# Hansard-T/FHE-Linformer

Measured on AMD Instinct MI355X. Metric: encrypted Linformer-d128 forward ms/sample, lower is better.
Workload: dtype u64

## Files before the change

### fhe-linformer_amd/csrc/context.cpp

```cpp
#include "context.h"
#include <hip/hip_runtime.h>
#include <algorithm>
#include <cstdio>
#include <cstdlib>
#include <cstring>
#include <sys/random.h>
#include <time.h>
#include <cxxabi.h>
#include <dlfcn.h>
#include <execinfo.h>

namespace fhelin {

void hip_check(hipError_t e, const char* what) {
    if (e != hipSuccess) throw Error(FHELIN_ERR_HIP, std::string(what) + ": " + hipGetErrorString(e));
}

void* DevicePool::raw_malloc(size_t bytes) {
    if (backend_.malloc_fn) return backend_.malloc_fn(bytes);
    void* p = nullptr;
    if (hipMalloc(&p, bytes) != hipSuccess) {
        (void)hipGetLastError();
        return nullptr;
    }
// ... 115 lines not shown
    sl.free_at.erase(off);
    if (len > bytes) {
        sl.free_at[off + bytes] = len - bytes;
        ln.by_size.emplace(len - bytes, std::make_pair(slab, off + bytes));
    }
    sl.used += bytes;
    void* p = sl.base + off;
    live_[p] = Live{bytes, cur_lane, slab, off};
    live_bytes_ += bytes;
    if (live_bytes_ > live_peak) live_peak = live_bytes_;
    return p;
}
void DevicePool::free(void* p, unsigned used_by_lanes) {
    if (!p) return;
    auto it = live_.find(p);
    if (it == live_.end()) throw Error(FHELIN_ERR_STATE, "DevicePool::free of unknown pointer");
    const Live lv = it->second;
    live_.erase(it);
    live_bytes_ -= lv.bytes;
    Lane& ln = lane_[lv.lane];
    ln.slabs[lv.slab].used -= lv.bytes;
    unsigned wait = used_by_lanes;
    if (have_streams && lv.lane != cur_lane) {
        wait |= 1u << cur_lane;
        if (conservative_foreign_free)
            for (int k = 0; k <= n_user_lanes; ++k) wait |= 1u << k;
    }
    wait &= ~(1u << lv.lane);
    if (!have_streams || !wait) {
        insert_free(ln, lv.slab, lv.off, lv.bytes);
        return;
    }
    Parked pk{lv.slab, lv.off, lv.bytes, {}, 0};
    for (int k = 0; k < MAX_LANES; ++k) {
        if (!(wait & (1u << k)) || !lane_stream[k]) continue;
        hipEvent_t ev = nullptr;
        if (!spare_events_.empty()) {
            ev = spare_events_.back();
            spare_events_.pop_back();
        } else {
            hip_check(hipEventCreateWithFlags(&ev, hipEventDisableTiming), "hipEventCreate(pool)");
        }
        hip_check(hipEventRecord(ev, lane_stream[k]), "hipEventRecord(pool free)");
        pk.ev[pk.n_ev++] = ev;
    }
    foreign_frees += 1;
    ln.parked.push_back(pk);
}
void DevicePool::trim() {
    trims += 1;
    if (!backend_.malloc_fn) (void)hipDeviceSynchronize();
    for (auto& ln : lane_) {
        for (auto& pk : ln.parked) {
            for (int k = 0; k < pk.n_ev; ++k) spare_events_.push_back(pk.ev[k]);
            insert_free(ln, pk.slab, pk.off, pk.len);
        }
        ln.parked.clear();
        for (size_t i = 0; i < ln.slabs.size(); ++i) {
            Slab& sl = ln.slabs[i];
            if (!sl.base || sl.used != 0) continue;
            erase_size_entry(ln, (int)i, 0, sl.size);
            raw_free(sl.base);
            reserved_ -= sl.size;
            sl = Slab();
        }
    }
}

template <class T>
const T* Context::upload_table(const std::vector<T>& v) {
    void* p = nullptr;
    size_t bytes = std::max<size_t>(v.size() * sizeof(T), 16);
    hip_check(hipMalloc(&p, bytes), "hipMalloc(table)");
    if (!v.empty()) hip_check(hipMemcpy(p, v.data(), v.size() * sizeof(T), hipMemcpyHostToDevice), "hipMemcpy(table)");
    table_allocs.push_back(p);
    return static_cast<const T*>(p);
}
template const u64* Context::upload_table<u64>(const std::vector<u64>&);
template const int* Context::upload_table<int>(const std::vector<int>&);
template const u32* Context::upload_table<u32>(const std::vector<u32>&);
template const double* Context::upload_table<double>(const std::vector<double>&);

static u64 mont_r(u64 m) { return (u64)((((u128)1) << 64) % m); }

static u64 prod_mod(const std::vector<u64>& ms, int skip, u64 t) {
    u64 r = 1 % t;
    for (int i = 0; i < (int)ms.size(); ++i)
        if (i != skip) r = h_mulmod(r, ms[i] % t, t);
    return r;
}

static void resolve_seed(Params& p) {
    if (p.have_seed_bytes) return;
    if (p.seed != 0) {
        std::memset(p.seed_bytes, 0, sizeof p.seed_bytes);
        for (int i = 0; i < 8; ++i) p.seed_bytes[i] = (uint8_t)(p.seed >> (8 * i));
    } else {
        size_t got = 0;
        while (got < sizeof p.seed_bytes) {
            const ssize_t n = getrandom(p.seed_bytes + got, sizeof p.seed_bytes - got, 0);
            if (n <= 0) throw Error(FHELIN_ERR_INTERNAL, "getrandom failed: no entropy for key generation");
            got += (size_t)n;
        }
    }
    p.have_seed_bytes = true;
}

static Params resolve_params(Params p) {
    resolve_seed(p);
    if (p.n_p < 0 && p.n_q >= 1 && p.dnum >= 1 && p.special_bits >= 1) {
        const int a = (p.n_q + p.dnum - 1) / p.dnum;
        const int first = p.first_bits + (std::min(a, p.n_q) - 1) * p.scale_bits;
        const int other = p.n_q > a ? std::min(a, p.n_q - a) * p.scale_bits : 0;
        p.n_p = (std::max(first, other) + p.special_bits - 1) / p.special_bits;
    }
    return p;
}

Context::Context(const Params& p_in) : prm(resolve_params(p_in)) {
    const Params& p = prm;
    if (p.log_n < 12 || p.log_n > 17) throw Error(FHELIN_ERR_ARG, "log_n must be in [12,17]");
    if (p.n_q < 1 || p.n_q > 64 || p.n_p < 0 || p.n_p > 16) throw Error(FHELIN_ERR_ARG, "bad limb counts");
    if (p.dnum < 1) throw Error(FHELIN_ERR_ARG, "dnum must be >= 1");
    if (p.first_bits > 60 || p.scale_bits > 60 || p.special_bits > 60) throw Error(FHELIN_ERR_ARG, "primes must be <= 60 bits");
    if (p.first_bits < 20 || p.scale_bits < 20 || (p.n_p > 0 && p.special_bits < 20)) throw Error(FHELIN_ERR_ARG, "primes must be >= 20 bits");
    if (p.log_slots < 1 || p.log_slots > p.log_n - 1) throw Error(FHELIN_ERR_ARG, "log_slots out of range");
    N = 1 << p.log_n;
    L = p.n_q - 1;
    K = p.n_p;
    alpha = (p.n_q + p.dnum - 1) / p.dnum;
    if (alpha > 16) throw Error(FHELIN_ERR_ARG, "digit size > 16 limbs not supported");
    if ((p.n_q + alpha - 1) / alpha > 16) throw Error(FHELIN_ERR_ARG, "more than 16 key-switching digits not supported");
    try {
        chain = make_prime_chain(p.log_n, p.n_q, p.first_bits, p.scale_bits, p.n_p, p.special_bits);
    } catch (const std::exception& e) {
        throw Error(FHELIN_ERR_ARG, std::string("prime chain: ") + e.what());
    }
    moduli = chain.q;
    moduli.insert(moduli.end(), chain.p.begin(), chain.p.end());
    for (u64 q : moduli)
        if (q >> 60) throw Error(FHELIN_ERR_ARG, "prime chain: a modulus is >= 2^60 (lower scale_bits or first_bits)");
    for (u64 q : moduli) {
        barrett.push_back(h_barrett(q));
        tw.push_back(make_twiddles(q, p.log_n));
    }
    sf_real.assign(p.n_q + 1, 0.0L);
    sf_real[0] = (long double)chain.q[L];
    for (int k = 0; k < L; ++k) sf_real[k + 1] = sf_real[k] * sf_real[k] / (long double)chain.q[L - k];

    if (p.device < 0) return;

    int ndev = 0;
    if (hipGetDeviceCount(&ndev) != hipSuccess || ndev <= 0)
        throw Error(FHELIN_ERR_NO_DEVICE, "no HIP device visible: the fhe-linformer_amd engine has no CPU fallback");
    if (p.device >= ndev) throw Error(FHELIN_ERR_ARG, "device index out of range");
    hip_check(hipSetDevice(p.device), "hipSetDevice");
    hip_check(hipStreamCreateWithFlags(&stream, hipStreamNonBlocking), "hipStreamCreate");
    main_stream = stream;
    own_stream = true;
    {
        int want = 2;
        if (const char* e = std::getenv("FHELIN_LANES")) want = std::atoi(e);
        n_lanes = std::max(0, std::min(want, DevicePool::MAX_LANES - 1));
        for (int k = 1; k <= n_lanes; ++k) {
            hip_check(hipStreamCreateWithFlags(&lane_stream[k], hipStreamNonBlocking), "hipStreamCreate(lane)");
            hip_check(hipEventCreateWithFlags(&lane_event[k], hipEventDisableTiming), "hipEventCreate(lane)");
        }
        hip_check(hipEventCreateWithFlags(&fork_event, hipEventDisableTiming), "hipEventCreate(fork)");
        pool.lane_stream[0] = main_stream;
        for (int k = 1; k <= n_lanes; ++k) pool.lane_stream[k] = lane_stream[k];
        pool.have_streams = true;
        if (const char* e = std::getenv("FHELIN_ASYNC")) async_lanes = std::atoi(e) != 0;
        if (const char* e = std::getenv("FHELIN_FUSE_MODDOWN")) fuse_moddown = std::atoi(e) != 0;
        if (const char* e = std::getenv("FHELIN_FUSE_FINISH")) fuse_finish = std::atoi(e) != 0;
        if (const char* e = std::getenv("FHELIN_HOST_ENCODE")) host_encode = std::atoi(e) != 0;
        if (const char* e = std::getenv("FHELIN_FUSE_GATHER")) fuse_gather = std::atoi(e) != 0;
        if (const char* e = std::getenv("FHELIN_FUSE_LIFT")) fuse_lift = std::atoi(e) != 0;
        if (const char* e = std::getenv("FHELIN_LDS_DIGITS")) lds_digits = std::atoi(e) != 0;
        if (const char* e = std::getenv("FHELIN_NTT_TRACE")) trace_small_ntt = std::atoi(e);
        if (const char* e = std::getenv("FHELIN_HOST_WAITS")) trace_waits = std::atoi(e) != 0;
    }
    hip_check(hipEventCreate(&ev_start), "hipEventCreate");
    stage_words = (size_t)2 << p.log_n;
    for (int i = 0; i < STAGE_SLOTS; ++i) {
        hip_check(hipHostMalloc(reinterpret_cast<void**>(&stage_buf[i]), stage_words * sizeof(u64), hipHostMallocDefault), "hipHostMalloc(stage)");
        hip_check(hipEventCreateWithFlags(&stage_ev[i], hipEventDisableTiming), "hipEventCreate(stage)");
    }
    hip_check(hipHostMalloc(reinterpret_cast<void**>(&small_buf), (size_t)SMALL_SLOTS * SMALL_WORDS * sizeof(u64), hipHostMallocDefault), "hipHostMalloc(stage, small)");
    for (int i = 0; i < SMALL_SLOTS; ++i) hip_check(hipEventCreateWithFlags(&small_ev[i], hipEventDisableTiming), "hipEventCreate(stage, small)");
    hip_check(hipEventCreate(&ev_stop), "hipEventCreate");
    has_device = true;

    const int nl = (int)moduli.size();
    {
        std::vector<u64> bar(2 * nl), ninv(8 * nl, 0);
        for (int i = 0; i < nl; ++i) {
            bar[2 * i] = barrett[i].r0;
            bar[2 * i + 1] = barrett[i].r1;
            ninv[8 * i] = tw[i].n_inv;
            ninv[8 * i + 1] = tw[i].n_inv_s;
            ninv[8 * i + 2] = tw[i].w1_n_inv;
            ninv[8 * i + 3] = tw[i].w1_n_inv_s;
            int bits = 0;
            while (bits < 64 && (moduli[i] >> bits)) ++bits;
            if (bits >= 12 && bits <= 60) {
                ninv[8 * i + 4] = (u64)(bits - 10);
                ninv[8 * i + 5] = (u64)((((u128)1) << (bits + 22)) / moduli[i]);
            }
        }
        dt.log_n = p.log_n;
        dt.n_limbs = nl;
        dt.moduli = upload_table(moduli);
        dt.barrett = upload_table(bar);
        {
            std::vector<u64> qi(nl);
            for (int i = 0; i < nl; ++i) {
                u64 x = moduli[i];
                for (int it = 0; it < 6; ++it) x *= 2 - moduli[i] * x;
                qi[i] = x;
            }
            dt.qinv = upload_table(qi);
            std::vector<u64> mr(2 * (size_t)nl);
            for (int i = 0; i < nl; ++i) {
                mr[2 * i] = mont_r(moduli[i]);
                mr[2 * i + 1] = h_shoup(mr[2 * i], moduli[i]);
            }
            dt.mont = upload_table(mr);
        }
        dt.ninv = upload_table(ninv);
        std::vector<u64> f((size_t)nl * 2 * N), g((size_t)nl * 2 * N);
        for (int i = 0; i < nl; ++i) {
            std::memcpy(&f[(size_t)i * 2 * N], tw[i].fwd.data(), sizeof(u64) * 2 * N);
            std::memcpy(&g[(size_t)i * 2 * N], tw[i].inv.data(), sizeof(u64) * 2 * N);
        }
        dt.tw_fwd = upload_table(f);
        dt.tw_inv = upload_table(g);
        const size_t tiles = N >> 12;
        const size_t per_limb = tiles * 15 * 256 * 2;
        for (int dir = 0; dir < 2; ++dir) {
            const std::vector<u64>& src = dir ? g : f;
            std::vector<u64> r((size_t)nl * per_limb);
            for (int i = 0; i < nl; ++i)
                for (size_t T = 0; T < tiles; ++T)
                    for (int kb = 0; kb < 4; ++kb)
                        for (int j = 0; j < (8 >> kb); ++j)
                            for (size_t tau = 0; tau < 256; ++tau) {
                                const size_t idx = (N >> (kb + 1)) + ((((T << 8) | tau)) << (3 - kb)) + j;
                                const size_t s_ = (size_t)(8 >> kb) - 1 + j;
                                const size_t o = (size_t)i * per_limb + ((T * 15 + s_) * 256 + tau) * 2;
                                r[o] = src[(size_t)i * 2 * N + 2 * idx];
                                r[o + 1] = src[(size_t)i * 2 * N + 2 * idx + 1];
                            }
            (dir ? dt.tw_rows_inv : dt.tw_rows_fwd) = upload_table(r);
        }
    }
    {
        std::vector<u64> phatinv(2 * std::max(K, 1)), phatmod((size_t)std::max(K, 1) * (L + 1)), pinv(2 * (L + 1));
        for (int j = 0; j < K; ++j) {
            u64 pj = chain.p[j];
            u64 hat = prod_mod(chain.p, j, pj);
            u64 inv = h_invmod(hat, pj);
            phatinv[2 * j] = inv;
            phatinv[2 * j + 1] = h_shoup(inv, pj);
            for (int t = 0; t <= L; ++t) phatmod[(size_t)j * (L + 1) + t] = pack30(h_mulmod(prod_mod(chain.p, j, chain.q[t]), mont_r(chain.q[t]), chain.q[t]));
        }
        for (int t = 0; t <= L; ++t) {
            u64 qt = chain.q[t];
            u64 pm = prod_mod(chain.p, -1, qt);
            u64 inv = K > 0 ? h_invmod(pm, qt) : 1;
            pinv[2 * t] = inv;
            pinv[2 * t + 1] = h_shoup(inv, qt);
        }
        d_phatinv = upload_table(phatinv);
        d_phatmod = upload_table(phatmod);
        d_pinv = upload_table(pinv);
        std::vector<u64> pmod(2 * (L + 1));
        for (int t = 0; t <= L; ++t) {
            pmod[2 * t] = prod_mod(chain.p, -1, chain.q[t]);
            pmod[2 * t + 1] = h_shoup(pmod[2 * t], chain.q[t]);
        }
        d_pmod = upload_table(pmod);
        std::vector<u64> qlinv((size_t)(L + 1) * (L + 1) * 2, 0), qlmod((size_t)(L + 1) * (L + 1), 0);
        for (int l = 0; l <= L; ++l)
            for (int t = 0; t < l; ++t) {
                u64 qt = chain.q[t];
                u64 r = chain.q[l] % qt;
                u64 inv = h_invmod(r, qt);
                qlmod[(size_t)l * (L + 1) + t] = r;
                qlinv[((size_t)l * (L + 1) + t) * 2] = inv;
                qlinv[((size_t)l * (L + 1) + t) * 2 + 1] = h_shoup(inv, qt);
            }
        d_qlinv = upload_table(qlinv);
        d_qlmod = upload_table(qlmod);
    }
    lvl.resize(L + 2);
    for (int ell = 1; ell <= L + 1; ++ell) {
        LevelTables& lt = lvl[ell];
        lt.ell = ell;
        lt.beta = digits_at(ell);
        const int nt = ell + K;
        std::vector<u64> hatinv(2 * ell), hatmod((size_t)ell * nt, 0), hatmod2((size_t)ell * nt, 0);
        std::vector<int> tab((size_t)lt.beta * nt, -1);
        for (int j = 0; j < lt.beta; ++j) {
            const int lo = j * alpha, hi = std::min((j + 1) * alpha, ell);
            std::vector<u64> dig(chain.q.begin() + lo, chain.q.begin() + hi);
            for (int i = lo; i < hi; ++i) {
                u64 qi = chain.q[i];
                u64 inv = h_invmod(prod_mod(dig, i - lo, qi), qi);
                hatinv[2 * i] = inv;
                hatinv[2 * i + 1] = h_shoup(inv, qi);
                for (int t = 0; t < nt; ++t) {
                    u64 mt = t < ell ? chain.q[t] : chain.p[t - ell];
                    const u64 hr = h_mulmod(prod_mod(dig, i - lo, mt), mont_r(mt), mt);
                    hatmod[(size_t)i * nt + t] = pack30(hr);
                    hatmod2[(size_t)i * nt + t] = pack30(h_mulmod(hr, mont_r(mt), mt));
                }
            }
            for (int t = 0; t < nt; ++t) {
                bool own = t >= lo && t < hi;
                tab[(size_t)j * nt + t] = own ? -1 : (t < ell ? limb_id_q(t) : limb_id_p(t - ell));
            }
        }
        lt.up_hatinv = upload_table(hatinv);
        lt.up_hatmod = upload_table(hatmod);
        lt.up_hatmod_r2 = upload_table(hatmod2);
        lt.ext_limb_tab = upload_table(tab);
        if (ell >= 2 && K >= 1) {
            const u64 ql = chain.q[ell - 1];
            const int e1 = ell - 1;
            std::vector<u64> mhi(2 * (K + 1)), mhm((size_t)(K + 1) * e1), minv(2 * e1), mmod(e1);
            for (int j = 0; j <= K; ++j) {
                const u64 b = j < K ? chain.p[j] : ql;
                const u64 hat_b = j < K ? h_mulmod(prod_mod(chain.p, j, b), ql % b, b) : prod_mod(chain.p, -1, b);
                const u64 inv = h_invmod(hat_b, b);
                mhi[2 * j] = inv;
                mhi[2 * j + 1] = h_shoup(inv, b);
                for (int t = 0; t < e1; ++t) {
                    const u64 qt = chain.q[t];
                    mhm[(size_t)j * e1 + t] = pack30(j < K ? h_mulmod(prod_mod(chain.p, j, qt), ql % qt, qt) : prod_mod(chain.p, -1, qt));
                }
            }
            for (int t = 0; t < e1; ++t) {
                const u64 qt = chain.q[t];
                mmod[t] = h_mulmod(prod_mod(chain.p, -1, qt), ql % qt, qt);
                const u64 inv = h_invmod(mmod[t], qt);
                minv[2 * t] = inv;
                minv[2 * t + 1] = h_shoup(inv, qt);
            }
            lt.md_hatinv = upload_table(mhi);
            lt.md_hatmod = upload_table(mhm);
            lt.md_minv = upload_table(minv);
            lt.md_mmod = upload_table(mmod);
        }
    }
}

void Context::upload_async(u64* dst, const u64* src, size_t words) {
    if (words <= SMALL_WORDS && small_buf) {
        const int i = small_next;
        small_next = (small_next + 1) % SMALL_SLOTS;
        if (small_used[i]) {
            timespec a, b;
            if (trace_waits) clock_gettime(CLOCK_MONOTONIC, &a);
            hip_check(hipEventSynchronize(small_ev[i]), "hipEventSynchronize(stage, small)");
            if (trace_waits) {
                clock_gettime(CLOCK_MONOTONIC, &b);
                note_wait("upload ring (small)", (u64)((b.tv_sec - a.tv_sec) * 1000000000ll + (b.tv_nsec - a.tv_nsec)));
            }
        }
        u64* slot = small_buf + (size_t)i * SMALL_WORDS;
        std::memcpy(slot, src, words * sizeof(u64));
        hip_check(hipMemcpyAsync(dst, slot, words * sizeof(u64), hipMemcpyHostToDevice, stream), "hipMemcpyAsync(stage, small)");
        hip_check(hipEventRecord(small_ev[i], stream), "hipEventRecord(stage, small)");
        small_used[i] = true;
        return;
    }
    if (words > stage_words) throw Error(FHELIN_ERR_INTERNAL, "upload_async: block larger than a staging slot");
    const int i = stage_next;
    stage_next = (stage_next + 1) % STAGE_SLOTS;
    if (stage_used[i]) {
        timespec a, b;
        if (trace_waits) clock_gettime(CLOCK_MONOTONIC, &a);
        hip_check(hipEventSynchronize(stage_ev[i]), "hipEventSynchronize(stage)");
        if (trace_waits) {
            clock_gettime(CLOCK_MONOTONIC, &b);
            note_wait("upload ring (large)", (u64)((b.tv_sec - a.tv_sec) * 1000000000ll + (b.tv_nsec - a.tv_nsec)));
        }
    }
    std::memcpy(stage_buf[i], src, words * sizeof(u64));
    hip_check(hipMemcpyAsync(dst, stage_buf[i], words * sizeof(u64), hipMemcpyHostToDevice, stream), "hipMemcpyAsync(stage)");
    hip_check(hipEventRecord(stage_ev[i], stream), "hipEventRecord(stage)");
    stage_used[i] = true;
}

Context::~Context() {
    if (trace_waits) {
        fprintf(stderr, "[fhelin] host time blocked inside the library, by site (waits, ms):\n");
        for (const auto& e : wait_sites) fprintf(stderr, "  %8llu %10.1f  %s\n", (unsigned long long)e.second.first, e.second.second / 1e6, e.first.c_str());
    }
    if (trace_small_ntt && !small_ntt_sites.empty()) {
        std::vector<std::pair<std::string, std::pair<u64, u64>>> v(small_ntt_sites.begin(), small_ntt_sites.end());
        std::sort(v.begin(), v.end(), [](const auto& a, const auto& b) { return a.second.first > b.second.first; });
        fprintf(stderr, "[fhelin] transforms of <= %d limb vectors by call stack (launch pairs, limb vectors):\n", trace_small_ntt);
        for (size_t i = 0; i < v.size() && i < 40; ++i)
            fprintf(stderr, "  %8llu %9llu  %s\n", (unsigned long long)v[i].second.first, (unsigned long long)v[i].second.second, v[i].first.c_str());
    }
    if (has_device) {
        (void)hipSetDevice(prm.device);
        (void)hipDeviceSynchronize();
        for (void* p : table_allocs) (void)hipFree(p);
        for (int k = 1; k <= n_lanes; ++k) {
            if (lane_event[k]) (void)hipEventDestroy(lane_event[k]);
            if (lane_stream[k]) (void)hipStreamDestroy(lane_stream[k]);
        }
        if (fork_event) (void)hipEventDestroy(fork_event);
        for (int i = 0; i < STAGE_SLOTS; ++i) {
            if (stage_ev[i]) (void)hipEventDestroy(stage_ev[i]);
            if (stage_buf[i]) (void)hipHostFree(stage_buf[i]);
        }
        for (int i = 0; i < SMALL_SLOTS; ++i)
            if (small_ev[i]) (void)hipEventDestroy(small_ev[i]);
        if (small_buf) (void)hipHostFree(small_buf);
        if (ev_start) (void)hipEventDestroy(ev_start);
        if (ev_stop) (void)hipEventDestroy(ev_stop);
        if (own_stream && main_stream) (void)hipStreamDestroy(main_stream);
    }
}

void Context::require_device() const {
    if (!has_device)
        throw Error(FHELIN_ERR_NO_DEVICE, "operation needs the HIP device path (host-only context): no CPU fallback exists");
}
// ... 106 lines not shown
```

### fhe-linformer_amd/csrc/context.h

```cpp
#pragma once
#include <cstdint>
#include <map>
#include <memory>
#include <stdexcept>
#include <string>
#include <unordered_map>
#include <vector>
#include <hip/hip_runtime_api.h>
#include "../../include/fhelin.h"
#include "hostmath.h"
#include "kernels.h"

namespace fhelin {

struct Params {
    int log_n = 16;
    int n_q = 24;
    int first_bits = 55;
    int scale_bits = 52;
    int n_p = 6;
    int special_bits = 60;
    int dnum = 4;
    int log_slots = 14;
    int hamming = 192;
    uint64_t seed = 0;
    uint8_t seed_bytes[32] = {};
    bool have_seed_bytes = false;
    int device = 0;
};

struct Error : std::runtime_error {
    int code;
    Error(int c, const std::string& m) : std::runtime_error(m), code(c) {}
};

void hip_check(hipError_t e, const char* what);

class DevicePool {
public:
    static constexpr int MAX_LANES = 5;
    static constexpr size_t SLAB_MAX = size_t(8) << 30, SLAB_MIN = size_t(32) << 20;
    struct Backend {
        void* (*malloc_fn)(size_t) = nullptr;
        void (*free_fn)(void*) = nullptr;
    };
    DevicePool() = default;
    explicit DevicePool(const Backend& b) : backend_(b) {}
    ~DevicePool();
    void* alloc(size_t bytes);
    void free(void* p, unsigned used_by_lanes = 0);
    bool conservative_foreign_free = false;
    int n_user_lanes = 0;
    void trim();
    size_t bytes_reserved() const { return reserved_; }
    size_t bytes_live() const { return live_bytes_; }
    size_t slabs() const;
    size_t free_ranges() const;
    int cur_lane = 0;
    hipStream_t lane_stream[MAX_LANES] = {};
    bool have_streams = false;
    u64 malloc_calls = 0, malloc_bytes = 0, malloc_ns = 0;
    u64 foreign_frees = 0;
    u64 trims = 0;
    size_t live_peak = 0, reserved_peak = 0;
private:
    struct Slab {
        char* base = nullptr;
        size_t size = 0, used = 0;
        std::map<size_t, size_t> free_at;
    };
    struct Live { size_t bytes; int lane; int slab; size_t off; };
    struct Parked { int slab; size_t off, len; hipEvent_t ev[MAX_LANES]; int n_ev; };
    struct Lane {
        std::vector<Slab> slabs;
        std::multimap<size_t, std::pair<int, size_t>> by_size;
        std::vector<Parked> parked;
    };
    Backend backend_;
    Lane lane_[MAX_LANES];
    std::unordered_map<void*, Live> live_;
    std::vector<hipEvent_t> spare_events_;
    size_t reserved_ = 0, live_bytes_ = 0;
    void insert_free(Lane& ln, int slab, size_t off, size_t len);
    void erase_size_entry(Lane& ln, int slab, size_t off, size_t len);
    bool grow(Lane& ln, size_t bytes);
    void* raw_malloc(size_t bytes);
    void raw_free(void* p);
};

struct LevelTables {
    int ell = 0;
    int beta = 0;
    const u64* up_hatinv = nullptr;
    const u64* up_hatmod = nullptr;
    const u64* up_hatmod_r2 = nullptr;
    const int* ext_limb_tab = nullptr;
    const u64* md_hatinv = nullptr;
    const u64* md_hatmod = nullptr;
    const u64* md_minv = nullptr;
    const u64* md_mmod = nullptr;
};

struct OpStats {
    u64 limb_ntt = 0;
    u64 keyswitch = 0;
    u64 keyswitch_limbs = 0;
    u64 rescale = 0;
    u64 ct_pt_mult = 0;
    u64 bootstrap = 0;
    u64 encode = 0;
    u64 rescale_limbs = 0;
    u64 ct_pt_limbs = 0;
};

struct Context {
    Params prm;
    OpStats stats;
    int N = 0;
    int L = 0;
    int K = 0;
    int alpha = 0;
    PrimeChain chain;
    std::vector<u64> moduli;
    std::vector<Barrett> barrett;
    std::vector<TwiddleTable> tw;
    std::vector<long double> sf_real;

    bool has_device = false;
    hipStream_t stream = nullptr;
    hipStream_t main_stream = nullptr;
    bool own_stream = false;
    int n_lanes = 0;
    hipStream_t lane_stream[DevicePool::MAX_LANES] = {};
    hipEvent_t lane_event[DevicePool::MAX_LANES] = {};
    hipEvent_t fork_event = nullptr;
    bool async_lanes = true;
    int async_rr = 0;
    u64 lane_seq[DevicePool::MAX_LANES] = {};
    std::vector<std::pair<u64, std::shared_ptr<void>>> lane_hold[DevicePool::MAX_LANES];
    void release_holds(int lane, u64 up_to_seq);
    void fork_lanes();
    void join_lanes();
    struct LaneScope {
        Context& c;
        LaneScope(Context& ctx, int k) : c(ctx) {
            c.stream = c.lane_stream[k];
            c.pool.cur_lane = k;
        }
        ~LaneScope() {
            c.stream = c.main_stream;
            c.pool.cur_lane = 0;
        }
    };
    DevicePool pool;
    DeviceTables dt{};
    std::vector<void*> table_allocs;
    hipEvent_t ev_start = nullptr, ev_stop = nullptr;

    static constexpr int STAGE_SLOTS = 64;
    u64* stage_buf[STAGE_SLOTS] = {};
    hipEvent_t stage_ev[STAGE_SLOTS] = {};
    bool stage_used[STAGE_SLOTS] = {};
    int stage_next = 0;
    size_t stage_words = 0;
    static constexpr int SMALL_SLOTS = 256;
    static constexpr size_t SMALL_WORDS = 8192;
    u64* small_buf = nullptr;
    hipEvent_t small_ev[SMALL_SLOTS] = {};
    bool small_used[SMALL_SLOTS] = {};
    int small_next = 0;
    void upload_async(u64* dst, const u64* src, size_t words);

    const u64* d_phatinv = nullptr;
    const u64* d_phatmod = nullptr;
    const u64* d_pinv = nullptr;
    const u64* d_pmod = nullptr;
    const u64* d_qlinv = nullptr;
    const u64* d_qlmod = nullptr;
    std::vector<LevelTables> lvl;
    std::map<u64, const u32*> automorph_maps;

    explicit Context(const Params& p);
    ~Context();
    Context(const Context&) = delete;
    Context& operator=(const Context&) = delete;

    void require_device() const;
    template <class T> T* dalloc(size_t count) { return static_cast<T*>(pool.alloc(count * sizeof(T))); }
    template <class T> const T* upload_table(const std::vector<T>& v);
    int limb_id_q(int i) const { return i; }
    int limb_id_p(int j) const { return L + 1 + j; }
    int digits_at(int ell) const { return (ell + alpha - 1) / alpha; }
    u64 galois_element(int rot_index) const;
    const u32* automorph_map(u64 galois);
    const u32* automorph_inverse_of(const u32* map);
    std::map<const u32*, const u32*> automorph_inverse;
    bool fuse_finish = true;
    bool fuse_moddown = false;
    bool host_encode = false;
    bool fuse_gather = true;
    bool fuse_lift = true;
    bool lds_digits = true;
    struct FftDev {
        const u32* rot = nullptr;
        const double* ksi = nullptr;
    };
    std::map<int, FftDev> fft_dev;
    void sync();
    void ntt(const LimbBatch& b, bool inverse, int active = -1) {
        stats.limb_ntt += (u64)(active >= 0 ? active : b.nvec);
        if (trace_small_ntt && b.nvec <= trace_small_ntt) note_small_ntt(b.nvec);
        launch_ntt(dt, b, inverse, stream);
    }
    bool trace_waits = false;
    std::map<std::string, std::pair<u64, u64>> wait_sites;
    void note_wait(const char* site, u64 ns) {
        auto& e = wait_sites[site];
        e.first += 1;
        e.second += ns;
    }
    int trace_small_ntt = 0;
    std::map<std::string, std::pair<u64, u64>> small_ntt_sites;
    void note_small_ntt(int nvec);
    void ntt_epilogue(const LimbBatch& b, const NttEpilogue& ep) {
        stats.limb_ntt += (u64)b.nvec;
        if (trace_small_ntt && b.nvec <= trace_small_ntt) note_small_ntt(b.nvec);
        launch_ntt_epilogue(dt, b, ep, stream);
    }
};

}
```

### fhe-linformer_amd/csrc/evaluator.cpp

```cpp
#include "evaluator.h"
#include <map>
#include <hip/hip_runtime.h>
#include <cmath>
#include <cstring>

namespace fhelin {

DevBlock::~DevBlock() {
    if (d && ctx) {
        try { ctx->pool.free(d); } catch (...) {}
    }
}
Ciphertext::~Ciphertext() {
    if (async_ev) (void)hipEventDestroy(async_ev);
    if (d && ctx && !block) {
        try { ctx->pool.free(d); } catch (...) {}
    }
}
Encoding::~Encoding() {
    if (ready) (void)hipEventDestroy(ready);
    if (d && ctx) {
        try { ctx->pool.free(d, lanes_ordered); } catch (...) {}
    }
}
// ... 61 lines not shown

std::vector<CtPtr> Evaluator::make_contiguous(const std::vector<CtPtr>& v, int site) {
    if (v.size() <= 1 || contiguous_base(v)) return v;
    if (site >= 0 && site < 8) gather_copies[site] += v.size();
    std::vector<CtPtr> o = new_ct_batch((int)v.size(), v[0]->npoly, v[0]->ell, v[0]->deg, v[0]->scale, v[0]->slots);
    for (size_t lo = 0; lo < v.size(); lo += EwItems::MAX_ITEMS) {
        EwItems it;
        it.n = (int)std::min<size_t>(EwItems::MAX_ITEMS, v.size() - lo);
        it.vecs = v[0]->npoly * v[0]->ell;
        it.b_vecs = 0;
        for (int i = 0; i < it.n; ++i) {
            if (v[lo + i]->words() != v[0]->words()) throw Error(FHELIN_ERR_INTERNAL, "make_contiguous: operands of different shapes");
            it.out[i] = o[lo + i]->d;
            it.a[i] = v[lo + i]->d;
            it.b[i] = nullptr;
        }
        launch_ew_items(c_.dt, it, 4, v[0]->ell, c_.stream);
    }
    hip_check(hipGetLastError(), "batch gather");
    return o;
}

KeyPtr Evaluator::new_key() {
    c_.require_device();
    auto k = std::make_shared<EvalKey>();
    k->ctx = &c_;
    k->digits = c_.digits_at(c_.L + 1);
    k->d = c_.dalloc<u64>(k->words());
    return k;
}

void Evaluator::keyswitch(const u64* c_ntt, int ell, const EvalKey& key, u64* out, const u64* add0, const u64* add1,
                          const u32* map, const u64* post) {
    keyswitch_batch(1, c_ntt, 0, ell, key, out, 0, add0, add1, 0, map, post, 0);
}

void Evaluator::keyswitch_batch(int B, const u64* c_ntt, size_t c_stride, int ell, const EvalKey& key, u64* out, size_t out_stride,
                                const u64* add0, const u64* add1, size_t add_stride, const u32* map, const u64* post,
                                size_t post_stride) {
    keyswitch_impl(B, nullptr, c_ntt, c_stride, ell, &key, out, out_stride, add0, add1, add_stride, map, post, post_stride);
}

void Evaluator::keyswitch_rows(const KsRows& rows, const u64* c_ntt, size_t c_stride, int ell, u64* out, size_t out_stride,
                               const u64* add0, size_t add_stride) {
    const int B = (int)rows.keys.size();
    if (B < 1) return;
    if (B > KsShape::MAX_ROWS || rows.maps.size() != rows.keys.size()) throw Error(FHELIN_ERR_ARG, "keyswitch_rows: bad row count");
    keyswitch_impl(B, &rows, c_ntt, c_stride, ell, nullptr, out, out_stride, add0, nullptr, add_stride, nullptr, nullptr, 0);
}

void Evaluator::keyswitch_impl(int B, const KsRows* rows, const u64* c_ntt, size_t c_stride, int ell, const EvalKey* key, u64* out,
                               size_t out_stride, const u64* add0, const u64* add1, size_t add_stride, const u32* map, const u64* post,
                               size_t post_stride) {
    c_.require_device();
    if (c_.K < 1) throw Error(FHELIN_ERR_STATE, "hybrid key switching needs at least one special prime");
    if (B < 1) return;
    const size_t N = c_.N;
    const int K = c_.K, L1 = c_.L + 1;
    const LevelTables& lt = c_.lvl[ell];
    const int nt = ell + K;
    KsShape sh{ell, K, c_.alpha, lt.beta, L1, B, c_stride, out_stride, add_stride, post_stride};
    const bool shared = rows && rows->shared_input;
    if (rows) {
        sh.per_row = 1;
        sh.shared_input = shared ? 1 : 0;
        for (int b = 0; b < B; ++b) {
            sh.evk_row[b] = rows->keys[b]->d;
            sh.map_row[b] = rows->maps[b];
        }
    }
    const int Bu = shared ? 1 : B;
    KsShape shu = sh;
    shu.batch = Bu;
    hipStream_t s = c_.stream;
    u64* cc = c_.dalloc<u64>((size_t)Bu * ell * N);
    c_.stats.keyswitch += (u64)B;
    c_.stats.keyswitch_limbs += (u64)B * ell;
    {
        LimbBatch ib{cc, Bu * ell, nullptr, 0, ell, c_ntt};
        if (Bu > 1 && c_stride != (size_t)ell * N) {
            ib.src_group = ell;
            ib.src_group_stride = c_stride;
        }
        c_.ntt(ib, true);
    }
    u64* ext = c_.dalloc<u64>((size_t)Bu * lt.beta * nt * N);
    launch_modup_conv(c_.dt, shu, ext, cc, c_ntt, lt.up_hatinv, lt.up_hatmod_r2, s);
    LimbBatch eb{ext, Bu * lt.beta * nt, lt.ext_limb_tab, 0, 1};
    eb.tab_len = lt.beta * nt;
    eb.lazy_out = true;
    c_.ntt(eb, false, Bu * (lt.beta * nt - ell));
    u64* accQ = c_.dalloc<u64>((size_t)B * 2 * ell * N);
    u64* accP = c_.dalloc<u64>((size_t)B * 2 * K * N);
    launch_ks_inner(c_.dt, sh, accQ, accP, ext, key ? key->d : nullptr, c_ntt, s);
    c_.ntt(LimbBatch{accP, B * 2 * K, nullptr, L1, K}, true);
    u64* conv = c_.dalloc<u64>((size_t)B * 2 * ell * N);
    launch_moddown_conv(c_.dt, sh, conv, accP, c_.d_phatinv, c_.d_phatmod, s);
    const bool identity = !map && !rows;
    if (c_.fuse_moddown || (c_.fuse_finish && identity)) {
        NttEpilogue ep;
        ep.acc = accQ;
        ep.acc_poly_stride = (size_t)ell * N;
        ep.out = out;
        ep.out_stride = out_stride;
        ep.w = c_.d_pinv;
        ep.ell = ell;
        ep.add0 = add0;
        ep.add1 = add1;
        ep.add_stride = add_stride;
        ep.post = post;
        ep.post_stride = post_stride;
        if (rows) {
            ep.per_row = 1;
            for (int b = 0; b < B; ++b) ep.invmap_row[b] = c_.automorph_inverse_of(rows->maps[b]);
        } else if (map) {
            ep.invmap = c_.automorph_inverse_of(map);
        }
        c_.ntt_epilogue(LimbBatch{conv, B * 2 * ell, nullptr, 0, ell}, ep);
    } else {
        c_.ntt(LimbBatch{conv, B * 2 * ell, nullptr, 0, ell}, false);
        launch_moddown_finish(c_.dt, sh, out, accQ, conv, c_.d_pinv, add0, add1, map, post, s);
    }
    launch_ok("keyswitch");
    c_.pool.free(cc);
    c_.pool.free(ext);
    c_.pool.free(accQ);
    c_.pool.free(accP);
    c_.pool.free(conv);
}

void Evaluator::moddown_rescale_finish(const KsShape& sh, u64* out, const u64* accQ, u64* conv, const u64* minv) {
    const int e1 = sh.ell - 1;
    const LimbBatch cb{conv, sh.batch * 2 * e1, nullptr, 0, e1};
    if (c_.fuse_finish) {
        NttEpilogue ep;
        ep.acc = accQ;
        ep.acc_poly_stride = (size_t)sh.ell * c_.N;
        ep.out = out;
        ep.out_stride = sh.out_stride;
        ep.w = minv;
        ep.ell = e1;
        c_.ntt_epilogue(cb, ep);
        return;
    }
    c_.ntt(cb, false);
    launch_moddown_rescale_finish(c_.dt, sh, out, accQ, conv, minv, c_.stream);
}

bool Evaluator::have_rotation_keys(const std::vector<int>& indices, int slots) const {
    const int ns = slots > 0 ? slots : (1 << c_.prm.log_slots);
    for (int r : indices) {
        if (r % ns == 0) return false;
        if (!rot_keys.count(c_.galois_element(r))) return false;
    }
    return !indices.empty();
}

const u64* Evaluator::permuted(const EvalKey& key, const u32* map) {
    if (key.d_perm) return key.d_perm;
    const int nvec = key.digits * 2 * (c_.L + 1 + c_.K);
    key.d_perm = c_.dalloc<u64>(key.words());
    launch_automorph_pack30(c_.dt, key.d_perm, key.d, map, nvec, c_.stream);
    launch_ok("key permutation");
    hip_check(hipStreamSynchronize(c_.stream), "key permutation sync");
    return key.d_perm;
}

std::vector<CtPtr> Evaluator::rotate_sum_batch(const std::vector<CtPtr>& vin, const std::vector<int>& indices) {
    if (vin.empty()) return {};
    const int R = (int)indices.size();
    if (R < 1 || R > KsShape::MAX_ROT) throw Error(FHELIN_ERR_ARG, "rotate_sum_batch: 1..7 rotations");
    if (!have_rotation_keys(indices, vin[0]->slots)) throw Error(FHELIN_ERR_KEY, "rotate_sum_batch: missing rotation key");
    if (c_.K < 1) throw Error(FHELIN_ERR_STATE, "hybrid key switching needs at least one special prime");
    std::vector<const EvalKey*> keys;
    std::vector<const u32*> maps;
    for (int r : indices) {
        const u64 g = c_.galois_element(r);
        keys.push_back(rot_keys.at(g).get());
        maps.push_back(c_.automorph_map(g));
    }
    const size_t N = c_.N;
    const int K = c_.K, L1 = c_.L + 1;
    hipStream_t s = c_.stream;
    std::vector<CtPtr> out(vin.size());
    std::vector<char> done(vin.size(), 0);
    for (size_t first = 0; first < vin.size(); ++first) {
        if (done[first]) continue;
        if (vin[first]->npoly != 2) throw Error(FHELIN_ERR_STATE, "rotate: ciphertext must have 2 components");
        std::vector<size_t> idx;
        for (size_t i = first; i < vin.size() && (int)idx.size() < batch_limit; ++i) {
            const CtPtr &a = vin[first], &b = vin[i];
            if (!done[i] && b->npoly == 2 && b->ell == a->ell && b->deg == a->deg && fabsl(b->scale / a->scale - 1.0L) < 1e-9L)
                idx.push_back(i);
        }
        std::vector<CtPtr> chunk;
        for (size_t i : idx) chunk.push_back(vin[i]);
        chunk = make_contiguous(chunk, 0);
        const int B = (int)chunk.size(), ell = chunk[0]->ell;
        const size_t pn = (size_t)ell * N, ctw = 2 * pn;
        const LevelTables& lt = c_.lvl[ell];
        const int nt = ell + K;
        std::vector<CtPtr> o = new_ct_batch(B, 2, ell, chunk[0]->deg, chunk[0]->scale, chunk[0]->slots);
        const u64* base = chunk[0]->d;
        KsShape sh{ell, K, c_.alpha, lt.beta, L1, B, ctw, ctw, pn, ctw};
        sh.n_rot = R;
        sh.lds_digits = c_.lds_digits ? 1 : 0;
        for (int r = 0; r < R; ++r) {
            sh.evk_rot[r] = permuted(*keys[r], maps[r]);
            sh.map_rot[r] = maps[r];
            if (c_.galois_element(indices[r]) % (u64)(c_.N / 256) != 1) sh.lds_digits = 0;
        }
        int steps = 0;
        while ((1 << steps) < R + 1) ++steps;
        c_.stats.keyswitch += (u64)B * steps;
        c_.stats.keyswitch_limbs += (u64)B * steps * ell;
        u64* cc = c_.dalloc<u64>((size_t)B * ell * N);
        {
            LimbBatch ib{cc, B * ell, nullptr, 0, ell, base + pn};
            if (B > 1) {
                ib.src_group = ell;
                ib.src_group_stride = ctw;
            }
            c_.ntt(ib, true);
        }
        u64* ext = c_.dalloc<u64>((size_t)B * lt.beta * nt * N);
        launch_modup_conv(c_.dt, sh, ext, cc, base + pn, lt.up_hatinv, lt.up_hatmod, s);
        LimbBatch eb{ext, B * lt.beta * nt, lt.ext_limb_tab, 0, 1};
        eb.tab_len = lt.beta * nt;
        eb.lazy_out = true;
        c_.ntt(eb, false, B * (lt.beta * nt - ell));
        u64* accQ = c_.dalloc<u64>((size_t)B * 2 * ell * N);
        u64* accP = c_.dalloc<u64>((size_t)B * 2 * K * N);
        launch_ks_inner_multi(c_.dt, sh, accQ, accP, ext, base + pn, s);
        u64* c0sum = nullptr;
        if (c_.fuse_gather) {
            sh.gsrc = base;
            sh.gsrc_stride = ctw;
        } else {
            c0sum = c_.dalloc<u64>((size_t)B * ell * N);
            launch_gather_sum(c_.dt, sh, c0sum, base, ctw, s);
        }
        c_.ntt(LimbBatch{accP, B * 2 * K, nullptr, L1, K}, true);
        u64* conv = c_.dalloc<u64>((size_t)B * 2 * ell * N);
        launch_moddown_conv(c_.dt, sh, conv, accP, c_.d_phatinv, c_.d_phatmod, s);
        c_.ntt(LimbBatch{conv, B * 2 * ell, nullptr, 0, ell}, false);
        launch_moddown_finish(c_.dt, sh, o[0]->d, accQ, conv, c_.d_pinv, c0sum, nullptr, nullptr, base, s);
        launch_ok("rotate_sum_batch");
        c_.pool.free(cc);
        c_.pool.free(ext);
        c_.pool.free(accQ);
        c_.pool.free(accP);
        if (c0sum) c_.pool.free(c0sum);
        c_.pool.free(conv);
        for (int b = 0; b < B; ++b) {
            o[b]->scale = vin[idx[b]]->scale;
            out[idx[b]] = o[b];
            done[idx[b]] = 1;
        }
    }
    return out;
}

Evaluator::FoldedKey Evaluator::folded_key(const PtPtr& p, int index, long double scale) {
    const u64 g = c_.galois_element(index);
    auto kit = rot_keys.find(g);
    if (kit == rot_keys.end()) throw Error(FHELIN_ERR_KEY, "no rotation key for index " + std::to_string(index) + " (EvalRotateKeyGen list)");
    for (size_t i = 0; i < folded_keys.size(); ++i) {
        const FoldedKey& f = folded_keys[i];
        if (f.pt.get() == p.get() && f.key.get() == kit->second.get() && f.index == index && f.scale == scale) {
            FoldedKey hit = f;
            if (i + 1 != folded_keys.size()) {
                folded_keys.erase(folded_keys.begin() + i);
                folded_keys.push_back(hit);
            }
            return hit;
        }
    }
    FoldedKey f;
    f.pt = p;
    f.key = kit->second;
    f.index = index;
    f.scale = scale;
    const int nl = c_.L + 1 + c_.K;
    f.enc = p->at(nl, scale);
    f.d = std::make_shared<DevBlock>();
    f.d->ctx = &c_;
    f.d->d = c_.dalloc<u64>(f.key->words());
    launch_fold_key(c_.dt, f.d->d, f.key->d, c_.automorph_map(g), f.enc->d, f.key->digits * 2 * nl, c_.stream);
    launch_ok("fold_key");
    hip_check(hipStreamSynchronize(c_.stream), "fold_key sync");
    if (folded_keys.size() >= MAX_FOLDED) {
        hip_check(hipStreamSynchronize(c_.main_stream), "folded key eviction sync");
        for (int k = 1; k <= c_.n_lanes; ++k) hip_check(hipStreamSynchronize(c_.lane_stream[k]), "folded key eviction sync (lane)");
        folded_keys.erase(folded_keys.begin());
    }
    folded_keys.push_back(f);
    return f;
}

std::vector<CtPtr> Evaluator::hoisted_dot_rows(const std::vector<CtPtr>& xin, const std::vector<PtPtr>& pts, const std::vector<int>& indices,
                                              bool rescale_out) {
    if (xin.empty()) return {};
    const int R = (int)indices.size();
    if (R < 1 || R > KsShape::MAX_ROT || (int)pts.size() != R + 1)
        throw Error(FHELIN_ERR_ARG, "hoisted_dot_rows: 1..7 rotations, one plaintext per rotation + the unrotated term's");
    if (!have_rotation_keys(indices, xin[0]->slots)) throw Error(FHELIN_ERR_KEY, "hoisted_dot_rows: missing rotation key");
    if (c_.K < 1) throw Error(FHELIN_ERR_STATE, "hybrid key switching needs at least one special prime");
    const int ns = xin[0]->slots > 0 ? xin[0]->slots : (1 << c_.prm.log_slots);
    for (int r : indices)
        if (r % ns == 0) throw Error(FHELIN_ERR_ARG, "hoisted_dot_rows: a rotation by 0 is the unrotated term (pts[0])");
    if (rescale_out && c_.K + 1 > 16)
        return rescale_batch(hoisted_dot_rows(xin, pts, indices, false));
    std::vector<CtPtr> x = xin;
    {
        std::vector<CtPtr> need;
        std::vector<size_t> pos;
        for (size_t i = 0; i < x.size(); ++i)
            if (x[i]->deg >= 2) {
                need.push_back(x[i]);
                pos.push_back(i);
            }
        if (!need.empty()) {
            std::vector<CtPtr> r = rescale_batch(need);
            for (size_t k = 0; k < pos.size(); ++k) x[pos[k]] = r[k];
        }
    }
    std::vector<const u32*> maps;
    for (int r : indices) maps.push_back(c_.automorph_map(c_.galois_element(r)));
    const size_t N = c_.N;
    const int K = c_.K, L1 = c_.L + 1;
    hipStream_t s = c_.stream;
    std::vector<CtPtr> out(x.size());
    std::vector<char> done(x.size(), 0);
    for (size_t first = 0; first < x.size(); ++first) {
        if (done[first]) continue;
        if (x[first]->npoly != 2) throw Error(FHELIN_ERR_STATE, "hoisted_dot_rows: ciphertext must have 2 components");
        std::vector<size_t> idx;
        for (size_t i = first; i < x.size() && (int)idx.size() < batch_limit; ++i) {
            const CtPtr &a = x[first], &b = x[i];
            if (!done[i] && b->npoly == 2 && b->ell == a->ell && b->deg == a->deg && fabsl(b->scale / a->scale - 1.0L) < 1e-9L) idx.push_back(i);
        }
        std::vector<CtPtr> chunk;
        for (size_t i : idx) chunk.push_back(x[i]);
        chunk = make_contiguous(chunk, 0);
        const int B = (int)chunk.size(), ell = chunk[0]->ell;
        const size_t pn = (size_t)ell * N, ctw = 2 * pn;
        const LevelTables& lt = c_.lvl[ell];
        const int nt = ell + K;
        const long double sf = c_.sf_real[chunk[0]->level()];
        const bool merged = rescale_out && ell >= 2 && K + 1 <= 16;
        if (rescale_out && !merged) throw Error(FHELIN_ERR_STATE, "hoisted_dot_rows: no limb left to drop");
        const int oell = merged ? ell - 1 : ell;
        std::vector<CtPtr> o = new_ct_batch(B, 2, oell, merged ? chunk[0]->deg : chunk[0]->deg + 1, chunk[0]->scale * sf, chunk[0]->slots);
        const u64* base = chunk[0]->d;
        KsShape sh{ell, K, c_.alpha, lt.beta, L1, B, ctw, (size_t)2 * oell * N, pn, ctw};
        sh.n_rot = R;
        sh.lds_digits = c_.lds_digits ? 1 : 0;
        HoistAdd h;
        h.n_rot = R;
        std::vector<FoldedKey> hold;
        const std::shared_ptr<Encoding> e0 = pts[0]->at(ell, sf);
        h.v[0] = e0->d;
        for (int r = 0; r < R; ++r) {
            hold.push_back(folded_key(pts[r + 1], indices[r], sf));
            sh.evk_rot[r] = hold.back().d->d;
            sh.map_rot[r] = maps[r];
            h.v[r + 1] = hold.back().enc->d;
            h.map[r] = maps[r];
            if (c_.galois_element(indices[r]) % (u64)(c_.N / 256) != 1) sh.lds_digits = 0;
        }
        c_.stats.keyswitch += (u64)B * R;
        c_.stats.keyswitch_limbs += (u64)B * R * ell;
        c_.stats.ct_pt_mult += (u64)B * (R + 1);
        c_.stats.ct_pt_limbs += (u64)B * (R + 1) * ell;
        if (merged) {
            c_.stats.rescale += (u64)B;
            c_.stats.rescale_limbs += (u64)B * ell;
        }
        u64* cc = c_.dalloc<u64>((size_t)B * ell * N);
        {
            LimbBatch ib{cc, B * ell, nullptr, 0, ell, base + pn};
            if (B > 1) {
                ib.src_group = ell;
                ib.src_group_stride = ctw;
            }
            c_.ntt(ib, true);
        }
        u64* ext = c_.dalloc<u64>((size_t)B * lt.beta * nt * N);
        launch_modup_conv(c_.dt, sh, ext, cc, base + pn, lt.up_hatinv, lt.up_hatmod, s);
        LimbBatch eb{ext, B * lt.beta * nt, lt.ext_limb_tab, 0, 1};
        eb.tab_len = lt.beta * nt;
        eb.lazy_out = true;
        c_.ntt(eb, false, B * (lt.beta * nt - ell));
        u64* accQ = c_.dalloc<u64>((size_t)B * 2 * ell * N);
        u64* accP = c_.dalloc<u64>((size_t)B * 2 * K * N);
        launch_ks_inner_multi(c_.dt, sh, accQ, accP, ext, base + pn, s);
        u64* pre = nullptr;
        u64* conv = nullptr;
        u64* top = nullptr;
        if (!merged) {
            pre = c_.dalloc<u64>((size_t)B * ctw);
            launch_hoist_addends(c_.dt, sh, h, pre, base, s);
            c_.ntt(LimbBatch{accP, B * 2 * K, nullptr, L1, K}, true);
            conv = c_.dalloc<u64>((size_t)B * 2 * ell * N);
            launch_moddown_conv(c_.dt, sh, conv, accP, c_.d_phatinv, c_.d_phatmod, s);
            c_.ntt(LimbBatch{conv, B * 2 * ell, nullptr, 0, ell}, false);
            launch_moddown_finish(c_.dt, sh, o[0]->d, accQ, conv, c_.d_pinv, nullptr, nullptr, nullptr, pre, s);
        } else {
            h.acc = accQ;
            h.pmod = c_.d_pmod;
            launch_hoist_addends(c_.dt, sh, h, nullptr, base, s);
            c_.ntt(LimbBatch{accP, B * 2 * K, nullptr, L1, K}, true);
            top = c_.dalloc<u64>((size_t)B * 2 * N);
            {
                LimbBatch tb{top, B * 2, nullptr, ell - 1, 1, accQ + (size_t)(ell - 1) * N};
                tb.src_group = 1;
                tb.src_group_stride = pn;
                c_.ntt(tb, true);
            }
            conv = c_.dalloc<u64>((size_t)B * 2 * (ell - 1) * N);
            launch_moddown_rescale_conv(c_.dt, sh, conv, accP, top, lt.md_hatinv, lt.md_hatmod, lt.md_mmod, s);
            moddown_rescale_finish(sh, o[0]->d, accQ, conv, lt.md_minv);
        }
        launch_ok("hoisted_dot_rows");
        c_.pool.free(cc);
        c_.pool.free(ext);
        c_.pool.free(accQ);
        c_.pool.free(accP);
        if (pre) c_.pool.free(pre);
        if (top) c_.pool.free(top);
        c_.pool.free(conv);
        for (int b = 0; b < B; ++b) {
            o[b]->scale = x[idx[b]]->scale * sf;
            if (merged) o[b]->scale = o[b]->scale / (long double)c_.chain.q[ell - 1];
            out[idx[b]] = o[b];
            done[idx[b]] = 1;
        }
    }
    return out;
}

CtPtr Evaluator::rotate_each_sum(const std::vector<CtPtr>& vin, const std::vector<int>& indices) {
    if (vin.empty() || vin.size() != indices.size()) throw Error(FHELIN_ERR_ARG, "rotate_each_sum: one index per ciphertext");
    const int ns = vin[0]->slots > 0 ? vin[0]->slots : (1 << c_.prm.log_slots);
    std::vector<CtPtr> rot;
    std::vector<int> ridx;
    CtPtr acc;
    for (size_t i = 0; i < vin.size(); ++i) {
        if (indices[i] % ns == 0) acc = acc ? add(acc, vin[i]) : vin[i];
        else {
            rot.push_back(vin[i]);
            ridx.push_back(indices[i]);
        }
    }
    for (size_t first = 0; first < rot.size(); first += KsShape::MAX_ROT) {
        const int R = (int)std::min(rot.size() - first, (size_t)KsShape::MAX_ROT);
        std::vector<CtPtr> chunk(rot.begin() + first, rot.begin() + first + R);
        bool uniform = have_rotation_keys(std::vector<int>(ridx.begin() + first, ridx.begin() + first + R), ns) && c_.K >= 1;
        for (const CtPtr& c : chunk)
            uniform = uniform && c->npoly == 2 && c->ell == chunk[0]->ell && c->deg == chunk[0]->deg &&
                      fabsl(c->scale / chunk[0]->scale - 1.0L) < 1e-9L;
        if (!uniform || R < 2) {
            for (int r = 0; r < R; ++r) {
                CtPtr t = rotate(chunk[r], ridx[first + r]);
                acc = acc ? add(acc, t) : t;
            }
            continue;
        }
        chunk = make_contiguous(chunk, 1);
        const size_t N = c_.N;
        const int K = c_.K, L1 = c_.L + 1, ell = chunk[0]->ell;
        const size_t pn = (size_t)ell * N, ctw = 2 * pn;
        const LevelTables& lt = c_.lvl[ell];
        const int nt = ell + K;
        hipStream_t s = c_.stream;
        const u64* base = chunk[0]->d;
        KsShape up{ell, K, c_.alpha, lt.beta, L1, R, ctw, 0, 0, 0};
        u64* cc = c_.dalloc<u64>((size_t)R * ell * N);
        {
            LimbBatch ib{cc, R * ell, nullptr, 0, ell, base + pn};
            ib.src_group = ell;
            ib.src_group_stride = ctw;
            c_.ntt(ib, true);
        }
        u64* ext = c_.dalloc<u64>((size_t)R * lt.beta * nt * N);
        launch_modup_conv(c_.dt, up, ext, cc, base + pn, lt.up_hatinv, lt.up_hatmod, s);
        LimbBatch eb{ext, R * lt.beta * nt, lt.ext_limb_tab, 0, 1};
        eb.tab_len = lt.beta * nt;
        eb.lazy_out = true;
        c_.ntt(eb, false, R * (lt.beta * nt - ell));
        KsShape sh{ell, K, c_.alpha, lt.beta, L1, 1, 0, ctw, pn, 0};
        sh.n_rot = R;
        sh.rot_ext_stride = (size_t)lt.beta * nt * N;
        sh.rot_input_stride = ctw;
        for (int r = 0; r < R; ++r) {
            const u64 g = c_.galois_element(ridx[first + r]);
            sh.map_rot[r] = c_.automorph_map(g);
            sh.evk_rot[r] = permuted(*rot_keys.at(g), sh.map_rot[r]);
        }
        c_.stats.keyswitch += (u64)R;
        c_.stats.keyswitch_limbs += (u64)R * ell;
        u64* accQ = c_.dalloc<u64>((size_t)2 * ell * N);
        u64* accP = c_.dalloc<u64>((size_t)2 * K * N);
        launch_ks_inner_multi(c_.dt, sh, accQ, accP, ext, base + pn, s);
        u64* c0sum = nullptr;
        if (c_.fuse_gather) {
            sh.gsrc = base;
            sh.gsrc_stride = 0;
        } else {
            c0sum = c_.dalloc<u64>((size_t)ell * N);
            launch_gather_sum(c_.dt, sh, c0sum, base, 0, s);
        }
        c_.ntt(LimbBatch{accP, 2 * K, nullptr, L1, K}, true);
        u64* conv = c_.dalloc<u64>((size_t)2 * ell * N);
        launch_moddown_conv(c_.dt, sh, conv, accP, c_.d_phatinv, c_.d_phatmod, s);
        c_.ntt(LimbBatch{conv, 2 * ell, nullptr, 0, ell}, false);
        CtPtr o = new_ct(2, ell, chunk[0]->deg, chunk[0]->scale, chunk[0]->slots);
        launch_moddown_finish(c_.dt, sh, o->d, accQ, conv, c_.d_pinv, c0sum, nullptr, nullptr, nullptr, s);
        launch_ok("rotate_each_sum");
        c_.pool.free(cc);
        c_.pool.free(ext);
        c_.pool.free(accQ);
        c_.pool.free(accP);
        if (c0sum) c_.pool.free(c0sum);
        c_.pool.free(conv);
        acc = acc ? add(acc, o) : o;
    }
    return acc;
}

std::vector<CtPtr> Evaluator::rotate_each_sum_rows(const std::vector<std::vector<CtPtr>>& rows, const std::vector<int>& indices) {
    if (rows.empty()) return {};
    const int ns = rows[0][0]->slots > 0 ? rows[0][0]->slots : (1 << c_.prm.log_slots);
    std::vector<int> rot_pos, plain_pos, ridx;
    for (size_t r = 0; r < indices.size(); ++r) {
        if (indices[r] % ns == 0) plain_pos.push_back((int)r);
        else {
            rot_pos.push_back((int)r);
            ridx.push_back(indices[r]);
        }
    }
    const int R = (int)rot_pos.size();
    bool uniform = R >= 2 && R <= KsShape::MAX_ROT && have_rotation_keys(ridx, ns) && c_.K >= 1;
    const CtPtr& f = rows[0][0];
    for (const auto& row : rows) {
        uniform = uniform && row.size() == indices.size();
        for (const CtPtr& c : row)
            uniform = uniform && c->npoly == 2 && c->ell == f->ell && c->deg == f->deg && fabsl(c->scale / f->scale - 1.0L) < 1e-9L;
    }
    std::vector<CtPtr> out(rows.size());
    if (!uniform) {
        for (size_t b = 0; b < rows.size(); ++b) out[b] = rotate_each_sum(rows[b], indices);
        return out;
    }
    const size_t N = c_.N;
    const int K = c_.K, L1 = c_.L + 1, ell = f->ell;
    const size_t pn = (size_t)ell * N, ctw = 2 * pn;
    const LevelTables& lt = c_.lvl[ell];
    const int nt = ell + K;
    hipStream_t s = c_.stream;
    const size_t chunk_rows = (size_t)std::max(1, batch_limit / 2);
    for (size_t lo = 0; lo < rows.size(); lo += chunk_rows) {
        const size_t hi = std::min(rows.size(), lo + chunk_rows);
        const int B = (int)(hi - lo);
        std::vector<CtPtr> flat;
        for (size_t b = lo; b < hi; ++b)
            for (int r : rot_pos) flat.push_back(rows[b][r]);
        size_t row_stride = (size_t)R * ctw;
        bool regular = B >= 1 && flat[0]->block != nullptr;
        for (int b = 0; b < B && regular; ++b) {
            for (int r = 0; r < R && regular; ++r) {
                const CtPtr& c = flat[(size_t)b * R + r];
                regular = c->block == flat[0]->block && c->words() == (size_t)ctw &&
                          c->d == flat[(size_t)b * R]->d + (size_t)r * ctw;
            }
            if (regular && b == 1) {
                regular = flat[R]->d > flat[0]->d;
                if (regular) row_stride = (size_t)(flat[R]->d - flat[0]->d);
            }
            if (regular && b >= 1) regular = flat[(size_t)b * R]->d == flat[0]->d + (size_t)b * row_stride;
        }
        if (!regular) {
            flat = make_contiguous(flat, 2);
            row_stride = (size_t)R * ctw;
        }
        const u64* base = flat[0]->d;
        KsShape up{ell, K, c_.alpha, lt.beta, L1, B * R, ctw, 0, 0, 0};
        u64* cc = c_.dalloc<u64>((size_t)B * R * ell * N);
        {
            LimbBatch ib{cc, B * R * ell, nullptr, 0, ell, base + pn};
            ib.src_group = ell;
            ib.src_group_stride = ctw;
            if (row_stride != (size_t)R * ctw) {
                ib.src_group2 = R;
                ib.src_group2_stride = row_stride;
            }
            c_.ntt(ib, true);
        }
        u64* ext = c_.dalloc<u64>((size_t)B * R * lt.beta * nt * N);
        launch_modup_conv(c_.dt, up, ext, cc, base + pn, lt.up_hatinv, lt.up_hatmod, s);
        LimbBatch eb{ext, B * R * lt.beta * nt, lt.ext_limb_tab, 0, 1};
        eb.tab_len = lt.beta * nt;
        eb.lazy_out = true;
        c_.ntt(eb, false, B * R * (lt.beta * nt - ell));
        KsShape sh{ell, K, c_.alpha, lt.beta, L1, B, row_stride, ctw, pn, 0};
        sh.n_rot = R;
        sh.rot_ext_stride = (size_t)lt.beta * nt * N;
        sh.rot_input_stride = ctw;
        sh.ext_batch_stride = (size_t)R * lt.beta * nt * N;
        for (int r = 0; r < R; ++r) {
            const u64 g = c_.galois_element(ridx[r]);
            sh.map_rot[r] = c_.automorph_map(g);
            sh.evk_rot[r] = permuted(*rot_keys.at(g), sh.map_rot[r]);
        }
        sh.gsrc = base;
        sh.gsrc_stride = row_stride;
        c_.stats.keyswitch += (u64)B * R;
        c_.stats.keyswitch_limbs += (u64)B * R * ell;
        u64* accQ = c_.dalloc<u64>((size_t)B * 2 * ell * N);
        u64* accP = c_.dalloc<u64>((size_t)B * 2 * K * N);
        launch_ks_inner_multi(c_.dt, sh, accQ, accP, ext, base + pn, s);
        c_.ntt(LimbBatch{accP, B * 2 * K, nullptr, L1, K}, true);
        u64* conv = c_.dalloc<u64>((size_t)B * 2 * ell * N);
        launch_moddown_conv(c_.dt, sh, conv, accP, c_.d_phatinv, c_.d_phatmod, s);
        c_.ntt(LimbBatch{conv, B * 2 * ell, nullptr, 0, ell}, false);
        std::vector<CtPtr> o = new_ct_batch(B, 2, ell, f->deg, f->scale, f->slots);
        launch_moddown_finish(c_.dt, sh, o[0]->d, accQ, conv, c_.d_pinv, nullptr, nullptr, nullptr, nullptr, s);
        launch_ok("rotate_each_sum_rows");
        c_.pool.free(cc);
        c_.pool.free(ext);
        c_.pool.free(accQ);
        c_.pool.free(accP);
        c_.pool.free(conv);
        for (int b = 0; b < B; ++b) out[lo + b] = o[b];
    }
    if (!plain_pos.empty()) {
        std::vector<CtPtr> acc(rows.size());
        for (size_t b = 0; b < rows.size(); ++b) acc[b] = rows[b][plain_pos[0]];
        for (size_t k = 1; k < plain_pos.size(); ++k) {
            std::vector<CtPtr> t(rows.size());
            for (size_t b = 0; b < rows.size(); ++b) t[b] = rows[b][plain_pos[k]];
            acc = add_batch(acc, t);
        }
        out = add_batch(acc, out);
    }
    return out;
}

std::vector<CtPtr> Evaluator::rotate_many(const CtPtr& a, const std::vector<int>& indices) {
    if (a->npoly != 2) throw Error(FHELIN_ERR_STATE, "rotate: ciphertext must have 2 components");
    const int ns = a->slots > 0 ? a->slots : (1 << c_.prm.log_slots);
    std::vector<CtPtr> out(indices.size());
    std::vector<size_t> todo;
    for (size_t i = 0; i < indices.size(); ++i) {
        if (indices[i] % ns == 0) out[i] = a;
        else todo.push_back(i);
    }
    const size_t pn = (size_t)a->ell * c_.N, ctw = 2 * pn;
    for (size_t first = 0; first < todo.size(); first += KsShape::MAX_ROWS) {
        const int B = (int)std::min(todo.size() - first, (size_t)KsShape::MAX_ROWS);
        if (B == 1) {
            out[todo[first]] = rotate(a, indices[todo[first]]);
            continue;
        }
        KsRows rows;
        rows.shared_input = true;
        for (int b = 0; b < B; ++b) {
            const int index = indices[todo[first + b]];
            const u64 g = c_.galois_element(index);
            auto it = rot_keys.find(g);
            if (it == rot_keys.end())
                throw Error(FHELIN_ERR_KEY, "no rotation key for index " + std::to_string(index) + " (EvalRotateKeyGen list)");
            rows.keys.push_back(it->second.get());
            rows.maps.push_back(c_.automorph_map(g));
        }
        std::vector<CtPtr> o = new_ct_batch(B, 2, a->ell, a->deg, a->scale, a->slots);
        keyswitch_rows(rows, a->d + pn, 0, a->ell, o[0]->d, ctw, a->d, 0);
        for (int b = 0; b < B; ++b) out[todo[first + b]] = o[b];
    }
    return out;
}

std::vector<CtPtr> Evaluator::rotate_each(const std::vector<CtPtr>& vin, const std::vector<int>& indices) {
    if (vin.size() != indices.size()) throw Error(FHELIN_ERR_ARG, "rotate_each: one index per ciphertext");
    std::vector<CtPtr> out(vin.size());
    std::vector<char> done(vin.size(), 0);
    for (size_t first = 0; first < vin.size(); ++first) {
        if (done[first]) continue;
        const CtPtr& a = vin[first];
        if (a->npoly != 2) throw Error(FHELIN_ERR_STATE, "rotate: ciphertext must have 2 components");
        const int ns = a->slots > 0 ? a->slots : (1 << c_.prm.log_slots);
        if (indices[first] % ns == 0) {
            out[first] = clone(a);
            done[first] = 1;
            continue;
        }
        std::vector<size_t> idx;
        for (size_t i = first; i < vin.size() && (int)idx.size() < std::min(batch_limit, (int)KsShape::MAX_ROWS); ++i) {
            const CtPtr& b = vin[i];
            if (!done[i] && indices[i] % ns != 0 && b->npoly == 2 && b->ell == a->ell && b->deg == a->deg &&
                fabsl(b->scale / a->scale - 1.0L) < 1e-9L)
                idx.push_back(i);
        }
        if (idx.size() < 2) {
            out[first] = rotate(a, indices[first]);
            done[first] = 1;
            continue;
// ... 124 lines not shown
    const u32* map = c_.automorph_map(g);
    std::vector<char> done(vin.size(), 0);
    for (size_t first = 0; first < vin.size(); ++first) {
        if (done[first]) continue;
        if (vin[first]->npoly != 2) throw Error(FHELIN_ERR_STATE, "rotate: ciphertext must have 2 components");
        std::vector<size_t> idx;
        for (size_t i = first; i < vin.size() && (int)idx.size() < batch_limit; ++i) {
            const CtPtr &a = vin[first], &b = vin[i];
            if (!done[i] && b->npoly == 2 && b->ell == a->ell && b->deg == a->deg && fabsl(b->scale / a->scale - 1.0L) < 1e-9L)
                idx.push_back(i);
        }
        std::vector<CtPtr> chunk;
        for (size_t i : idx) chunk.push_back(vin[i]);
        chunk = make_contiguous(chunk, 4);
        const int B = (int)chunk.size();
        const int ell = chunk[0]->ell;
        const size_t pn = (size_t)ell * c_.N, ctw = 2 * pn;
        std::vector<CtPtr> o = new_ct_batch(B, 2, ell, chunk[0]->deg, chunk[0]->scale, chunk[0]->slots);
        const u64* base = chunk[0]->d;
        keyswitch_batch(B, base + pn, ctw, ell, key, o[0]->d, ctw, base, nullptr, ctw, map, accumulate ? base : nullptr, ctw);
        for (int b = 0; b < B; ++b) {
            o[b]->scale = vin[idx[b]]->scale;
            out[idx[b]] = o[b];
            done[idx[b]] = 1;
        }
    }
    return out;
}

std::vector<std::vector<CtPtr>> Evaluator::rotate_many_batch(const std::vector<CtPtr>& xs, const std::vector<int>& indices) {
    std::vector<std::vector<CtPtr>> out(xs.size());
    if (xs.empty()) return out;
    bool uniform = xs.size() >= 2 && !c_.fuse_moddown && c_.K >= 1;
    for (const CtPtr& x : xs)
        uniform = uniform && x->npoly == 2 && x->ell == xs[0]->ell && x->deg == xs[0]->deg && x->slots == xs[0]->slots;
    if (!uniform) {
        for (size_t i = 0; i < xs.size(); ++i) out[i] = rotate_many(xs[i], indices);
        return out;
    }
    const int ns = xs[0]->slots > 0 ? xs[0]->slots : (1 << c_.prm.log_slots);
    std::vector<size_t> todo;
    for (size_t i = 0; i < xs.size(); ++i) out[i].resize(indices.size());
    for (size_t k = 0; k < indices.size(); ++k) {
        if (indices[k] % ns == 0)
            for (size_t i = 0; i < xs.size(); ++i) out[i][k] = xs[i];
        else
            todo.push_back(k);
    }
    const int R = (int)todo.size();
    if (R == 0) return out;
    std::vector<const EvalKey*> keys;
    std::vector<const u32*> maps;
    for (size_t k : todo) {
        const u64 g = c_.galois_element(indices[k]);
        auto it = rot_keys.find(g);
        if (it == rot_keys.end())
            throw Error(FHELIN_ERR_KEY, "no rotation key for index " + std::to_string(indices[k]) + " (EvalRotateKeyGen list)");
        keys.push_back(it->second.get());
        maps.push_back(c_.automorph_map(g));
    }
    const size_t N = c_.N;
    const int K = c_.K, L1 = c_.L + 1, ell = xs[0]->ell;
    const size_t pn = (size_t)ell * N, ctw = 2 * pn;
    const LevelTables& lt = c_.lvl[ell];
    const int nt = ell + K;
    hipStream_t s = c_.stream;
    const size_t per_pass = (size_t)std::max(1, 160 / R);
    for (size_t lo = 0; lo < xs.size(); lo += per_pass) {
        const size_t hi = std::min(xs.size(), lo + per_pass);
        const int B = (int)(hi - lo);
        std::vector<CtPtr> in = make_contiguous(std::vector<CtPtr>(xs.begin() + lo, xs.begin() + hi), 6);
        const u64* base = in[0]->d;
        const int rows = B * R;
        c_.stats.keyswitch += (u64)rows;
        c_.stats.keyswitch_limbs += (u64)rows * ell;
        KsShape up{ell, K, c_.alpha, lt.beta, L1, B, ctw, 0, 0, 0};
        u64* cc = c_.dalloc<u64>((size_t)B * ell * N);
        {
            LimbBatch ib{cc, B * ell, nullptr, 0, ell, base + pn};
            if (B > 1) {
                ib.src_group = ell;
                ib.src_group_stride = ctw;
            }
            c_.ntt(ib, true);
        }
        u64* ext = c_.dalloc<u64>((size_t)B * lt.beta * nt * N);
        launch_modup_conv(c_.dt, up, ext, cc, base + pn, lt.up_hatinv, lt.up_hatmod_r2, s);
        LimbBatch eb{ext, B * lt.beta * nt, lt.ext_limb_tab, 0, 1};
        eb.tab_len = lt.beta * nt;
        eb.lazy_out = true;
        c_.ntt(eb, false, B * (lt.beta * nt - ell));
        u64* accQ = c_.dalloc<u64>((size_t)rows * 2 * ell * N);
        u64* accP = c_.dalloc<u64>((size_t)rows * 2 * K * N);
        auto row_shape = [&](int first, int cnt) {
            KsShape sh{ell, K, c_.alpha, lt.beta, L1, B * cnt, ctw, ctw, ctw, 0};
            sh.per_row = 1;
            sh.shared_input = 1;
            sh.row_mod = cnt;
            sh.ext_batch_stride = (size_t)lt.beta * nt * N;
            for (int b = 0; b < cnt; ++b) {
                sh.evk_row[b] = keys[first + b]->d;
                sh.map_row[b] = maps[first + b];
            }
            return sh;
        };
        const bool one_chunk = R <= (int)KsShape::MAX_ROWS;
        if (one_chunk) launch_ks_inner(c_.dt, row_shape(0, R), accQ, accP, ext, nullptr, base + pn, s);
        else
            for (int i = 0; i < B; ++i)
                for (int first = 0; first < R; first += KsShape::MAX_ROWS) {
                    const int cnt = std::min(R - first, (int)KsShape::MAX_ROWS);
                    const size_t row0 = (size_t)i * R + first;
                    KsShape sh1{ell, K, c_.alpha, lt.beta, L1, cnt, 0, ctw, 0, 0};
                    sh1.per_row = 1;
                    sh1.shared_input = 1;
                    for (int b = 0; b < cnt; ++b) {
                        sh1.evk_row[b] = keys[first + b]->d;
                        sh1.map_row[b] = maps[first + b];
                    }
                    launch_ks_inner(c_.dt, sh1, accQ + row0 * 2 * ell * N, accP + row0 * 2 * K * N, ext + (size_t)i * lt.beta * nt * N, nullptr,
                                    base + pn + (size_t)i * ctw, s);
                }
        KsShape dn{ell, K, c_.alpha, lt.beta, L1, rows, 0, ctw, 0, 0};
        c_.ntt(LimbBatch{accP, rows * 2 * K, nullptr, L1, K}, true);
        u64* conv = c_.dalloc<u64>((size_t)rows * 2 * ell * N);
        launch_moddown_conv(c_.dt, dn, conv, accP, c_.d_phatinv, c_.d_phatmod, s);
        c_.ntt(LimbBatch{conv, rows * 2 * ell, nullptr, 0, ell}, false);
        std::vector<CtPtr> o = new_ct_batch(rows, 2, ell, xs[lo]->deg, xs[lo]->scale, xs[lo]->slots);
        if (one_chunk) {
            launch_moddown_finish(c_.dt, row_shape(0, R), o[0]->d, accQ, conv, c_.d_pinv, base, nullptr, nullptr, nullptr, s);
        } else {
            for (int i = 0; i < B; ++i)
                for (int first = 0; first < R; first += KsShape::MAX_ROWS) {
                    const int cnt = std::min(R - first, (int)KsShape::MAX_ROWS);
                    const size_t row0 = (size_t)i * R + first;
                    KsShape sh1{ell, K, c_.alpha, lt.beta, L1, cnt, 0, ctw, 0, 0};
                    sh1.per_row = 1;
                    sh1.shared_input = 1;
                    for (int b = 0; b < cnt; ++b) {
                        sh1.evk_row[b] = keys[first + b]->d;
                        sh1.map_row[b] = maps[first + b];
                    }
                    launch_moddown_finish(c_.dt, sh1, o[row0]->d, accQ + row0 * 2 * ell * N, conv + row0 * 2 * ell * N, c_.d_pinv,
                                          base + (size_t)i * ctw, nullptr, nullptr, nullptr, s);
                }
        }
        launch_ok("rotate_many_batch");
        c_.pool.free(cc);
        c_.pool.free(ext);
        c_.pool.free(accQ);
        c_.pool.free(accP);
        c_.pool.free(conv);
        for (int i = 0; i < B; ++i)
            for (int r = 0; r < R; ++r) {
                o[(size_t)i * R + r]->scale = xs[lo + i]->scale;
                out[lo + i][todo[r]] = o[(size_t)i * R + r];
            }
    }
    return out;
}

std::vector<CtPtr> Evaluator::rescale_batch(const std::vector<CtPtr>& vin) {
    std::vector<CtPtr> out(vin.size());
    std::vector<char> done(vin.size(), 0);
    for (size_t first = 0; first < vin.size(); ++first) {
        if (done[first]) continue;
        std::vector<size_t> idx;
        for (size_t i = first; i < vin.size() && (int)idx.size() < batch_limit; ++i)
            if (!done[i] && vin[i]->npoly == 2 && vin[first]->npoly == 2 && vin[i]->ell == vin[first]->ell) idx.push_back(i);
        if (idx.size() < 2) {
            out[first] = rescale(vin[first]);
            done[first] = 1;
            continue;
        }
        std::vector<CtPtr> chunk;
        for (size_t i : idx) chunk.push_back(vin[i]);
        chunk = make_contiguous(chunk, 5);
        const int B = (int)chunk.size(), ell = chunk[0]->ell, P = 2 * B;
        if (ell < 2) throw Error(FHELIN_ERR_STATE, "rescale: no limb left to drop");
        const size_t N = c_.N;
        const u64* base = chunk[0]->d;
        u64* last = c_.dalloc<u64>((size_t)P * N);
        c_.stats.rescale += (u64)B;
        c_.stats.rescale_limbs += (u64)B * ell;
        LimbBatch lb{last, P, nullptr, ell - 1, 1, base + (size_t)(ell - 1) * N};
        lb.src_group = 1;
        lb.src_group_stride = (size_t)ell * N;
        c_.ntt(lb, true);
        std::vector<CtPtr> o = new_ct_batch(B, 2, ell - 1, 1, 0, chunk[0]->slots);
        rescale_finish(o[0]->d, base, last, P, ell);
        launch_ok("rescale_batch");
        c_.pool.free(last);
        for (int b = 0; b < B; ++b) {
            const CtPtr& a = vin[idx[b]];
            o[b]->scale = a->scale / (long double)c_.chain.q[ell - 1];
            o[b]->deg = a->deg > 1 ? a->deg - 1 : 1;
            out[idx[b]] = o[b];
            done[idx[b]] = 1;
        }
    }
    return out;
}

std::vector<CtPtr> Evaluator::mult_plain_batch(const std::vector<CtPtr>& vin, const PtPtr& p) {
    return mult_plain_each(vin, std::vector<PtPtr>(vin.size(), p));
}

namespace {
template <class SameShape, class Emit>
// ... 60 lines not shown
    if (vin.size() != p.size() || vin.empty()) throw Error(FHELIN_ERR_ARG, "dot_plain: one plaintext per ciphertext, at least one term");
    std::vector<CtPtr> x = vin;
    {
        std::vector<CtPtr> need;
        std::map<const Ciphertext*, size_t> slot;
        for (size_t i = 0; i < vin.size(); ++i)
            if (vin[i]->deg >= 2 && !slot.count(vin[i].get())) {
                slot[vin[i].get()] = need.size();
                need.push_back(vin[i]);
            }
        if (!need.empty()) {
            std::vector<CtPtr> r = rescale_batch(need);
            for (size_t i = 0; i < vin.size(); ++i)
                if (vin[i]->deg >= 2) x[i] = r[slot[vin[i].get()]];
        }
    }
    bool uniform = x.size() >= 2;
    for (const CtPtr& c : x)
        uniform = uniform && c->npoly == x[0]->npoly && c->ell == x[0]->ell && c->deg == x[0]->deg && fabsl(c->scale / x[0]->scale - 1.0L) < 1e-9L;
    if (!uniform) {
        if (pt_scale > 0) throw Error(FHELIN_ERR_ARG, "dot_plain: an explicit plaintext scale needs uniform operands");
        std::vector<CtPtr> prod = mult_plain_each(x, p);
        CtPtr acc = prod[0];
        for (size_t i = 1; i < prod.size(); ++i) acc = add(acc, prod[i]);
        return acc;
    }
    const CtPtr& f = x[0];
    const long double sf = pt_scale > 0 ? pt_scale : c_.sf_real[f->level()];
    CtPtr acc;
    for (size_t lo = 0; lo < x.size(); lo += EwItems::MAX_ITEMS) {
        const size_t hi = std::min(x.size(), lo + (size_t)EwItems::MAX_ITEMS);
        EwItems it;
        it.n = (int)(hi - lo);
        it.vecs = f->npoly * f->ell;
        it.b_vecs = f->ell;
        for (size_t i = lo; i < hi; ++i) {
            it.a[i - lo] = x[i]->d;
            it.b[i - lo] = p[i]->at(f->ell, sf)->d;
        }
        const bool into_dest = dest && x.size() <= (size_t)EwItems::MAX_ITEMS && dest->npoly == f->npoly && dest->ell == f->ell;
        CtPtr o = into_dest ? dest : new_ct(f->npoly, f->ell, f->deg + 1, f->scale * sf, f->slots);
        if (into_dest) {
            o->deg = f->deg + 1;
            o->scale = f->scale * sf;
            o->slots = f->slots;
        }
        launch_ew_dot(c_.dt, o->d, it, f->ell, c_.stream);
        c_.stats.ct_pt_mult += (u64)(hi - lo);
        c_.stats.ct_pt_limbs += (u64)(hi - lo) * f->ell;
        acc = acc ? add(acc, o) : o;
    }
    launch_ok("dot_plain");
    return acc;
}

bool Evaluator::dot_plain_groups(const std::vector<CtPtr>& cts, const std::vector<std::vector<PtPtr>>& pts, long double pt_scale,
                                 const std::vector<CtPtr>& dest) {
    if (!dot_groups || cts.empty() || cts.size() > (size_t)EwDotGroups::MAX_A || pts.empty() || pts.size() > (size_t)EwDotGroups::MAX_G ||
        dest.size() != pts.size())
        return false;
    const CtPtr& f = cts[0];
    for (const CtPtr& c : cts)
        if (c->npoly != 2 || c->deg != 1 || c->ell != f->ell || fabsl(c->scale / f->scale - 1.0L) > 1e-9L) return false;
    for (const CtPtr& o : dest)
        if (!o || o->npoly != 2 || o->ell != f->ell) return false;
    const long double sf = pt_scale > 0 ? pt_scale : c_.sf_real[f->level()];
    EwDotGroups d;
    d.na = (int)cts.size();
    d.ng = (int)pts.size();
    d.ell = f->ell;
    for (int b = 0; b < d.na; ++b) d.a[b] = cts[b]->d;
    u64 terms = 0;
    for (int g = 0; g < d.ng; ++g) {
        if (pts[g].size() != cts.size()) return false;
        for (int b = 0; b < d.na; ++b) {
            d.p[g][b] = pts[g][b] ? pts[g][b]->at(f->ell, sf)->d : nullptr;
            terms += pts[g][b] ? 1 : 0;
        }
        d.out[g] = dest[g]->d;
        dest[g]->deg = f->deg + 1;
        dest[g]->scale = f->scale * sf;
        dest[g]->slots = f->slots;
    }
    launch_ew_dot_groups(c_.dt, d, c_.stream);
    launch_ok("dot_plain_groups");
    c_.stats.ct_pt_mult += terms;
    c_.stats.ct_pt_limbs += terms * (u64)f->ell;
    return true;
}

bool Evaluator::dot_plain_groups_batch(const std::vector<std::vector<CtPtr>>& cts, const std::vector<std::vector<PtPtr>>& pts, long double pt_scale,
                                       const std::vector<std::vector<CtPtr>>& dest) {
    const size_t nb = cts.size();
    if (!dot_groups || nb < 2 || dest.size() != nb || cts[0].empty() || cts[0].size() > (size_t)EwDotGroups::MAX_A || pts.empty() ||
        pts.size() > (size_t)EwDotGroups::MAX_G)
        return false;
    const size_t na = cts[0].size(), ng = pts.size();
    const CtPtr& f = cts[0][0];
    for (size_t x = 0; x < nb; ++x) {
        if (cts[x].size() != na || dest[x].size() != ng) return false;
        for (const CtPtr& c : cts[x])
            if (c->npoly != 2 || c->deg != 1 || c->ell != f->ell || fabsl(c->scale / f->scale - 1.0L) > 1e-9L) return false;
        for (const CtPtr& o : dest[x])
            if (!o || o->npoly != 2 || o->ell != f->ell) return false;
    }
    EwDotGroups d;
    d.na = (int)na;
    d.ng = (int)ng;
    d.ell = f->ell;
    d.nbatch = (int)nb;
    for (size_t b = 0; b < na; ++b) {
        if (cts[1][b]->d <= cts[0][b]->d) return false;
        const size_t st = (size_t)(cts[1][b]->d - cts[0][b]->d);
        for (size_t x = 0; x < nb; ++x)
            if (cts[x][b]->d != cts[0][b]->d + x * st) return false;
        d.a[b] = cts[0][b]->d;
        d.a_stride[b] = st;
    }
    for (size_t g = 0; g < ng; ++g) {
        if (dest[1][g]->d <= dest[0][g]->d) return false;
        const size_t st = (size_t)(dest[1][g]->d - dest[0][g]->d);
        for (size_t x = 0; x < nb; ++x)
            if (dest[x][g]->d != dest[0][g]->d + x * st) return false;
        d.out[g] = dest[0][g]->d;
        d.out_stride[g] = st;
    }
    const long double sf = pt_scale > 0 ? pt_scale : c_.sf_real[f->level()];
    u64 terms = 0;
    std::vector<std::shared_ptr<Encoding>> hold;
    for (size_t g = 0; g < ng; ++g) {
        if (pts[g].size() != na) return false;
        for (size_t b = 0; b < na; ++b) {
            if (pts[g][b]) {
                hold.push_back(pts[g][b]->at(f->ell, sf));
                d.p[g][b] = hold.back()->d;
                ++terms;
            } else {
                d.p[g][b] = nullptr;
            }
        }
        for (size_t x = 0; x < nb; ++x) {
            dest[x][g]->deg = f->deg + 1;
            dest[x][g]->scale = cts[x][0]->scale * sf;
            dest[x][g]->slots = f->slots;
        }
    }
    launch_ew_dot_groups(c_.dt, d, c_.stream);
    launch_ok("dot_plain_groups_batch");
    c_.stats.ct_pt_mult += terms * nb;
    c_.stats.ct_pt_limbs += terms * nb * (u64)f->ell;
    return true;
}

bool Evaluator::dot_plain_cyclic(const std::vector<CtPtr>& cts, const std::vector<PtPtr>& pts, const std::vector<CtPtr>& dest) {
    constexpr int P = EwCyclic::PERIOD;
    if (cts.empty() || (int)cts.size() > P || (int)pts.size() != P || (int)dest.size() != P) return false;
    const CtPtr& f = cts[0];
    for (const CtPtr& c : cts)
        if (c->npoly != 2 || c->deg != 1 || c->ell != f->ell || fabsl(c->scale / f->scale - 1.0L) > 1e-9L) return false;
    for (const CtPtr& o : dest)
        if (!o || o->npoly != 2 || o->ell != f->ell) return false;
    const long double sf = c_.sf_real[f->level()];
    EwCyclic d;
    d.n = (int)cts.size();
    d.ell = f->ell;
    std::vector<std::shared_ptr<Encoding>> hold;
    for (int j = 0; j < P; ++j) {
        hold.push_back(pts[j]->at(f->ell, sf));
        d.m[j] = hold.back()->d;
        d.a[j] = j < d.n ? cts[j]->d : nullptr;
        d.out[j] = dest[j]->d;
        dest[j]->deg = f->deg + 1;
        dest[j]->scale = f->scale * sf;
        dest[j]->slots = f->slots;
    }
    launch_ew_cyclic_dot(c_.dt, d, c_.stream);
    launch_ok("dot_plain_cyclic");
    c_.stats.ct_pt_mult += (u64)P * d.n;
    c_.stats.ct_pt_limbs += (u64)P * d.n * (u64)f->ell;
    return true;
}

bool Evaluator::dot_plain_window(const std::vector<CtPtr>& cur, const std::vector<CtPtr>& prev, const std::vector<PtPtr>& pts,
                                 const std::vector<CtPtr>& dest, bool accumulate) {
    constexpr int W = EwWindow::W;
    if ((int)cur.size() != W || (int)prev.size() != W || (int)pts.size() != W || (int)dest.size() != W) return false;
    CtPtr f;
    for (const auto* v : {&cur, &prev})
        for (const CtPtr& c : *v)
            if (c && !f) f = c;
    if (!f) return false;
    u64 terms = 0;
    for (const auto* v : {&cur, &prev})
        for (const CtPtr& c : *v)
            if (c) {
                if (c->npoly != 2 || c->deg != 1 || c->ell != f->ell || fabsl(c->scale / f->scale - 1.0L) > 1e-9L) return false;
                ++terms;
            }
    for (const CtPtr& o : dest)
        if (!o || o->npoly != 2 || o->ell != f->ell) return false;
    const long double sf = c_.sf_real[f->level()];
    EwWindow d;
    d.ell = f->ell;
    d.accumulate = accumulate ? 1 : 0;
    std::vector<std::shared_ptr<Encoding>> hold;
    for (int j = 0; j < W; ++j) {
        hold.push_back(pts[j]->at(f->ell, sf));
        d.m[j] = hold.back()->d;
        d.cur[j] = cur[j] ? cur[j]->d : dest[0]->d;
        d.prev[j] = prev[j] ? prev[j]->d : dest[0]->d;
        if (cur[j]) d.cur_mask |= 1u << j;
        if (prev[j]) d.prev_mask |= 1u << j;
        d.out[j] = dest[j]->d;
        dest[j]->deg = f->deg + 1;
        dest[j]->scale = f->scale * sf;
        dest[j]->slots = f->slots;
    }
    launch_ew_window_dot(c_.dt, d, c_.stream);
    launch_ok("dot_plain_window");
    c_.stats.ct_pt_mult += terms * (u64)W / 2;
    c_.stats.ct_pt_limbs += terms * (u64)W / 2 * (u64)f->ell;
    return true;
}

std::vector<CtPtr> Evaluator::add_batch(const std::vector<CtPtr>& a, const std::vector<CtPtr>& b) { return add_sub_batch(a, b, 1); }
std::vector<CtPtr> Evaluator::sub_batch(const std::vector<CtPtr>& a, const std::vector<CtPtr>& b) { return add_sub_batch(a, b, 2); }

void Evaluator::match_batch(const std::vector<CtPtr>& a, const std::vector<CtPtr>& b, std::vector<CtPtr>& x, std::vector<CtPtr>& y) {
    const size_t n = a.size();
// ... 114 lines not shown
        }
        std::vector<CtPtr> o = new_ct_batch(B, 2, ell, 2, 0, x[first]->slots);
        keyswitch_batch(B, d[0]->d + 2 * pn, 3 * pn, ell, *relin_key, o[0]->d, 2 * pn, d[0]->d, d[0]->d + pn, 3 * pn, nullptr, nullptr, 0);
        for (int k = 0; k < B; ++k) {
            const size_t i = idx[k];
            o[k]->deg = x[i]->deg + y[i]->deg;
            o[k]->scale = x[i]->scale * y[i]->scale;
            out[i] = o[k];
            done[i] = 1;
        }
    }
    launch_ok("mult_batch");
    return out;
}

std::vector<CtPtr> Evaluator::mult_affine_rescale_batch(const std::vector<CtPtr>& a, const std::vector<CtPtr>& b, int f, double cadd,
                                                        const std::vector<CtPtr>& sub) {
    if (a.size() != b.size() || (!sub.empty() && sub.size() != a.size())) throw Error(FHELIN_ERR_ARG, "mult_affine_rescale_batch: operand count mismatch");
    if (f != 1 && f != 2) throw Error(FHELIN_ERR_ARG, "mult_affine_rescale_batch: factor 1 or 2");
    if (!relin_key) throw Error(FHELIN_ERR_KEY, "no relinearisation key (EvalMultKeyGen not called)");
    if (c_.K < 1 || c_.K + 1 > 16) throw Error(FHELIN_ERR_STATE, "mult_affine_rescale_batch: 1..15 special primes");
    const size_t n = a.size();
    std::vector<CtPtr> in;
    std::map<const Ciphertext*, size_t> slot;
    for (const auto* side : {&a, &b})
        for (const CtPtr& c : *side) {
            if (c->npoly != 2) throw Error(FHELIN_ERR_STATE, "mult: operands must have 2 components");
            if (c->deg >= 2 && !slot.count(c.get())) {
                slot[c.get()] = in.size();
                in.push_back(c);
            }
        }
    std::vector<CtPtr> resc = in.empty() ? std::vector<CtPtr>() : rescale_batch(in);
    auto ready = [&](const CtPtr& c) { return c->deg >= 2 ? resc[slot[c.get()]] : c; };
    std::vector<CtPtr> x(n), y(n), out(n);
    for (size_t i = 0; i < n; ++i) match(ready(a[i]), ready(b[i]), x[i], y[i]);
    const size_t N = c_.N;
    const int K = c_.K, L1 = c_.L + 1;
    hipStream_t s = c_.stream;
    std::vector<char> done(n, 0);
    for (size_t first = 0; first < n; ++first) {
        if (done[first]) continue;
        std::vector<size_t> idx;
        for (size_t i = first; i < n && (int)idx.size() < batch_limit; ++i)
            if (!done[i] && x[i]->ell == x[first]->ell && fabsl(x[i]->scale * y[i]->scale / (x[first]->scale * y[first]->scale) - 1.0L) < 1e-12L)
                idx.push_back(i);
        const int B = (int)idx.size(), ell = x[first]->ell;
        if (ell < 2) throw Error(FHELIN_ERR_STATE, "mult_affine_rescale_batch: no limb left to drop");
        const size_t pn = (size_t)ell * N;
        const long double sc = x[first]->scale * y[first]->scale;
        const LevelTables& lt = c_.lvl[ell];
        const int nt = ell + K;
        std::vector<CtPtr> d = new_ct_batch(B, 3, ell, 2, 0, x[first]->slots);
        for (int k0 = 0; k0 < B; k0 += EwItems::MAX_ITEMS) {
            EwItems it;
            it.n = std::min(B - k0, (int)EwItems::MAX_ITEMS);
            for (int k = 0; k < it.n; ++k) {
                it.out[k] = d[k0 + k]->d;
                it.a[k] = x[idx[k0 + k]]->d;
                it.b[k] = y[idx[k0 + k]]->d;
            }
            launch_tensor_items(c_.dt, it, ell, s);
        }
        std::vector<CtPtr> sadj;
        if (!sub.empty()) {
            for (int k = 0; k < B; ++k) sadj.push_back(adjust(sub[idx[k]], ell, 2, sc));
            sadj = make_contiguous(sadj, 7);
        }
        ScalarSet cst;
        if (cadd != 0.0) real_to_scalars(c_, (long double)cadd * sc, ell, cst);
        KsShape sh{ell, K, c_.alpha, lt.beta, L1, B, 3 * pn, (size_t)2 * (ell - 1) * N, pn, 0};
        c_.stats.keyswitch += (u64)B;
        c_.stats.keyswitch_limbs += (u64)B * ell;
        c_.stats.rescale += (u64)B;
        c_.stats.rescale_limbs += (u64)B * ell;
        const u64* c_ntt = d[0]->d + 2 * pn;
        u64* cc = c_.dalloc<u64>((size_t)B * ell * N);
        {
            LimbBatch ib{cc, B * ell, nullptr, 0, ell, c_ntt};
            if (B > 1) {
                ib.src_group = ell;
                ib.src_group_stride = 3 * pn;
            }
            c_.ntt(ib, true);
        }
        u64* ext = c_.dalloc<u64>((size_t)B * lt.beta * nt * N);
        launch_modup_conv(c_.dt, sh, ext, cc, c_ntt, lt.up_hatinv, lt.up_hatmod_r2, s);
        LimbBatch eb{ext, B * lt.beta * nt, lt.ext_limb_tab, 0, 1};
        eb.tab_len = lt.beta * nt;
        eb.lazy_out = true;
        c_.ntt(eb, false, B * (lt.beta * nt - ell));
        u64* accQ = c_.dalloc<u64>((size_t)B * 2 * ell * N);
        u64* accP = c_.dalloc<u64>((size_t)B * 2 * K * N);
        launch_ks_inner(c_.dt, sh, accQ, accP, ext, relin_key->d, c_ntt, s);
        launch_affine_acc(c_.dt, sh, accQ, d[0]->d, sadj.empty() ? nullptr : sadj[0]->d, cst, cadd != 0.0 ? 1 : 0, f, c_.d_pmod, s);
        if (f == 2) launch_ew_add(c_.dt, accP, accP, accP, B * 2 * K, B * 2 * K, L1, K, s);
        c_.ntt(LimbBatch{accP, B * 2 * K, nullptr, L1, K}, true);
        u64* top = c_.dalloc<u64>((size_t)B * 2 * N);
        {
            LimbBatch tb{top, B * 2, nullptr, ell - 1, 1, accQ + (size_t)(ell - 1) * N};
            tb.src_group = 1;
            tb.src_group_stride = pn;
            c_.ntt(tb, true);
        }
        u64* conv = c_.dalloc<u64>((size_t)B * 2 * (ell - 1) * N);
        launch_moddown_rescale_conv(c_.dt, sh, conv, accP, top, lt.md_hatinv, lt.md_hatmod, lt.md_mmod, s);
        std::vector<CtPtr> o = new_ct_batch(B, 2, ell - 1, 1, 0, x[first]->slots);
        moddown_rescale_finish(sh, o[0]->d, accQ, conv, lt.md_minv);
        launch_ok("mult_affine_rescale_batch");
        c_.pool.free(cc);
        c_.pool.free(ext);
        c_.pool.free(accQ);
        c_.pool.free(accP);
        c_.pool.free(top);
        c_.pool.free(conv);
        for (int k = 0; k < B; ++k) {
            const size_t i = idx[k];
            o[k]->scale = x[i]->scale * y[i]->scale / (long double)c_.chain.q[ell - 1];
            out[i] = o[k];
            done[i] = 1;
        }
    }
    return out;
}

std::vector<CtPtr> Evaluator::add_plain_batch(const std::vector<CtPtr>& v, const PtPtr& p) {
    std::vector<CtPtr> out(v.size());
    for_runs(v.size(), [&](size_t a, size_t b) { return v[a]->npoly == v[b]->npoly && v[a]->ell == v[b]->ell; },
             [&](size_t lo, size_t hi) {
                 const CtPtr& f = v[lo];
                 std::vector<CtPtr> o = new_ct_batch((int)(hi - lo), f->npoly, f->ell, f->deg, f->scale, f->slots);
                 EwItems it;
                 it.n = (int)(hi - lo);
                 it.vecs = f->npoly * f->ell;
                 it.b_vecs = f->ell;
                 for (size_t i = lo; i < hi; ++i) {
                     auto enc = p->at(v[i]->ell, v[i]->scale);
                     o[i - lo]->deg = v[i]->deg;
                     o[i - lo]->scale = v[i]->scale;
                     it.out[i - lo] = o[i - lo]->d;
                     it.a[i - lo] = v[i]->d;
                     it.b[i - lo] = enc->d;
                     out[i] = o[i - lo];
                 }
                 launch_ew_items(c_.dt, it, 3, f->ell, c_.stream);
             });
    launch_ok("add_plain_batch");
    return out;
}

CtPtr Evaluator::rotate_add(const CtPtr& a, int index) {
    const int ns = a->slots > 0 ? a->slots : (1 << c_.prm.log_slots);
    if (index % ns == 0) return add(a, a);
    const u64 g = c_.galois_element(index);
    auto it = rot_keys.find(g);
    if (it == rot_keys.end())
        throw Error(FHELIN_ERR_KEY, "no rotation key for index " + std::to_string(index) + " (EvalRotateKeyGen list)");
    return raw_rotate(a, g, *it->second, true);
}

CtPtr Evaluator::raw_mult_relin(const CtPtr& a, const CtPtr& b, const EvalKey& key) {
    if (a->npoly != 2 || b->npoly != 2 || a->ell != b->ell) throw Error(FHELIN_ERR_STATE, "mult: operands must be 2-component, same level");
    const int ell = a->ell;
    const size_t pn = (size_t)ell * c_.N;
    u64* d = c_.dalloc<u64>(3 * pn);
    launch_tensor(c_.dt, d, a->d, b->d, ell, c_.stream);
    CtPtr o = new_ct(2, ell, a->deg + b->deg, a->scale * b->scale, a->slots);
    keyswitch(d + 2 * pn, ell, key, o->d, d, d + pn, nullptr);
    c_.pool.free(d);
    return o;
}

CtPtr Evaluator::raw_modraise(const CtPtr& a, int new_ell) {
    if (a->ell != 1) throw Error(FHELIN_ERR_STATE, "modraise: the input must have exactly one limb (q0)");
    if (new_ell < 1 || new_ell > c_.L + 1) throw Error(FHELIN_ERR_ARG, "modraise: bad target limb count");
    const size_t N = c_.N;
    const int P = a->npoly;
    hipStream_t s = c_.stream;
    u64* coef = c_.dalloc<u64>((size_t)P * N);
    LimbBatch ib{coef, P, nullptr, 0, 1, a->d};
    c_.ntt(ib, true);
    CtPtr up = new_ct(P, new_ell, a->deg, a->scale, a->slots);
    launch_modraise(c_.dt, up->d, coef, P, 0, new_ell, s);
    c_.ntt(LimbBatch{up->d, P * new_ell, nullptr, 0, new_ell}, false);
    launch_ok("modraise");
    c_.pool.free(coef);
    return up;
}

// ... 293 lines not shown
```

### fhe-linformer_amd/csrc/kernels.h

```cpp
#pragma once
#include <cstddef>
#include <cstdint>
#include <hip/hip_runtime_api.h>
#include "modarith.h"

namespace fhelin {

struct LimbBatch {
    u64* data;
    int nvec;
    const int* limb_tab;
    int limb_first;
    int limb_count;
    const u64* src = nullptr;
    int tab_len = 0;
    int src_group = 0;
    size_t src_group_stride = 0;
    int src_group2 = 0;
    size_t src_group2_stride = 0;
    bool lazy_out = false;
    const u64* lift_qlm = nullptr;
    int lift_limb = -1;
};

struct DeviceTables {
    int log_n;
    int n_limbs;
    const u64* moduli;
    const u64* barrett;
    const u64* qinv;
    const u64* mont;
    const u64* tw_fwd;
    const u64* tw_inv;
    const u64* tw_rows_fwd;
    const u64* tw_rows_inv;
    const u64* ninv;
};

struct NttEpilogue {
    static constexpr int MAX_ROWS = 16;
    const u64* acc = nullptr;
    size_t acc_poly_stride = 0;
    u64* out = nullptr;
    size_t out_stride = 0;
    const u64* w = nullptr;
    int ell = 0;
    const u64* add0 = nullptr;
    const u64* add1 = nullptr;
    const u64* post = nullptr;
    size_t add_stride = 0, post_stride = 0;
    const u32* invmap = nullptr;
    int per_row = 0;
    const u32* invmap_row[MAX_ROWS] = {};
};

void launch_ntt(const DeviceTables& t, const LimbBatch& b, bool inverse, hipStream_t s);
void launch_ntt_epilogue(const DeviceTables& t, const LimbBatch& b, const NttEpilogue& ep, hipStream_t s);


}
```

### fhe-linformer_amd/csrc/kernels_elem.h

```cpp
#pragma once
#include "kernels.h"

namespace fhelin {

struct ScalarSet {
    u64 v[128];
};

void launch_ew_mul(const DeviceTables& t, u64* out, const u64* a, const u64* b, int nvec, int b_mod, int limb_first, int limb_count, hipStream_t s);
void launch_ew_add(const DeviceTables& t, u64* out, const u64* a, const u64* b, int nvec, int b_mod, int limb_first, int limb_count, hipStream_t s);
void launch_ew_sub(const DeviceTables& t, u64* out, const u64* a, const u64* b, int nvec, int b_mod, int limb_first, int limb_count, hipStream_t s);
void launch_ew_muladd(const DeviceTables& t, u64* out, const u64* acc, const u64* a, const u64* b, int nvec, int b_mod, int limb_first,
                      int limb_count, hipStream_t s);
void launch_ew_neg(const DeviceTables& t, u64* out, const u64* a, int nvec, int limb_first, int limb_count, hipStream_t s);
void launch_ew_scalar(const DeviceTables& t, u64* out, const u64* a, const ScalarSet& sc, int nvec, int limb_first, int limb_count, hipStream_t s,
                      int in_limbs = 0);
void launch_ew_addscalar(const DeviceTables& t, u64* out, const u64* a, const ScalarSet& sc, int nvec, int limb_first, int limb_count, hipStream_t s,
                         int add_vecs = -1);
struct LinComb {
    static constexpr int MAX_TERMS = 32;
    int n = 0;
    int vecs = 0;
    const u64* a[MAX_TERMS];
};
void launch_ew_lincomb(const DeviceTables& t, u64* out, const LinComb& lc, const u64* scal, int ell, hipStream_t s, int in_limbs = 0);
void launch_tensor(const DeviceTables& t, u64* d, const u64* a, const u64* b, int ell, hipStream_t s);
struct EwItems;
void launch_tensor_items(const DeviceTables& t, const EwItems& it, int ell, hipStream_t s);
void launch_automorph(const DeviceTables& t, u64* out, const u64* in, const u32* map, int nvec, hipStream_t s);
void launch_automorph_pack30(const DeviceTables& t, u64* out, const u64* in, const u32* map, int nvec, hipStream_t s);
void launch_rescale_lift(const DeviceTables& t, u64* lifted, const u64* last, int npoly, int ell, const u64* qlmod_row, hipStream_t s);
void launch_rescale_finish(const DeviceTables& t, u64* out, const u64* c, const u64* lifted, int npoly, int ell, const u64* qlinv_row,
                           hipStream_t s);
void launch_modraise(const DeviceTables& t, u64* out, const u64* src, int npoly, int src_limb, int nl, hipStream_t s);
void launch_reduce_i128(const DeviceTables& t, u64* out, const u64* coeffs, int limb_first, int nlimbs, hipStream_t s);

struct EwItems {
    static constexpr int MAX_ITEMS = 32;
    int n = 0;
    int vecs = 0;
    int b_vecs = 0;
    u64* out[MAX_ITEMS];
    const u64* a[MAX_ITEMS];
    const u64* b[MAX_ITEMS];
};
void launch_ew_items(const DeviceTables& t, const EwItems& it, int op, int limb_count, hipStream_t s);
struct EwScaledDiff {
    static constexpr int MAX_ITEMS = 32;
    int n = 0;
    int vecs = 0;
    int ell = 0;
    u64* out[MAX_ITEMS];
    const u64* u[MAX_ITEMS];
    const u64* w[MAX_ITEMS];
};
void launch_ew_scaled_diff(const DeviceTables& t, const EwScaledDiff& d, const u64* consts, hipStream_t s);
void launch_ew_dot(const DeviceTables& t, u64* out, const EwItems& it, int limb_count, hipStream_t s);
struct EwDotGroups {
    static constexpr int MAX_A = 16, MAX_G = 8;
    int na = 0, ng = 0, ell = 0;
    const u64* a[MAX_A];
    const u64* p[MAX_G][MAX_A];
    u64* out[MAX_G];
    int nbatch = 1;
    size_t a_stride[MAX_A] = {};
    size_t out_stride[MAX_G] = {};
    u32 pmask[MAX_G] = {};
};
void launch_ew_dot_groups(const DeviceTables& t, const EwDotGroups& d, hipStream_t s);
struct EwCyclic {
    static constexpr int PERIOD = 32;
    int n = 0, ell = 0;
    const u64* a[PERIOD];
    const u64* m[PERIOD];
    u64* out[PERIOD];
};
void launch_ew_cyclic_dot(const DeviceTables& t, const EwCyclic& d, hipStream_t s);
struct EwWindow {
    static constexpr int W = 32;
    int ell = 0, accumulate = 0;
    u32 cur_mask = 0, prev_mask = 0;
    const u64* cur[W];
    const u64* prev[W];
    const u64* m[W];
    u64* out[W];
};
void launch_ew_window_dot(const DeviceTables& t, const EwWindow& d, hipStream_t s);

struct KsShape {
    int ell;
    int k;
    int alpha;
    int beta;
    int L1;
    int batch = 1;
    size_t c_stride = 0;
    size_t out_stride = 0;
    size_t add_stride = 0;
    size_t post_stride = 0;
    static constexpr int MAX_ROWS = 16;
    int per_row = 0;
    int shared_input = 0;
    int row_mod = 0;
    const u64* evk_row[MAX_ROWS] = {};
    const u32* map_row[MAX_ROWS] = {};
    static constexpr int MAX_ROT = 7;
    int n_rot = 0;
    const u64* evk_rot[MAX_ROT] = {};
    const u32* map_rot[MAX_ROT] = {};
    size_t rot_ext_stride = 0;
    size_t rot_input_stride = 0;
    int lds_digits = 0;
    size_t ext_batch_stride = 0;
    const u64* gsrc = nullptr;
    size_t gsrc_stride = 0;
    int tch = 16;
};
void launch_modup_conv(const DeviceTables& t, const KsShape& sh, u64* ext, const u64* cc, const u64* c_ntt, const u64* hatinv,
                       const u64* hatmod, hipStream_t s);
void launch_ks_inner(const DeviceTables& t, const KsShape& sh, u64* accQ, u64* accP, const u64* ext, const u64* evk, const u64* c_ntt,
                     hipStream_t s);
void launch_ks_inner_multi(const DeviceTables& t, const KsShape& sh, u64* accQ, u64* accP, const u64* ext, const u64* c_ntt,
                           hipStream_t s);
void launch_fold_key(const DeviceTables& t, u64* out, const u64* key, const u32* map, const u64* V, int nvec, hipStream_t s);
struct HoistAdd {
    int n_rot = 0;
    const u64* v[KsShape::MAX_ROT + 1] = {};
    const u32* map[KsShape::MAX_ROT] = {};
    u64* acc = nullptr;
    const u64* pmod = nullptr;
};
void launch_hoist_addends(const DeviceTables& t, const KsShape& sh, const HoistAdd& h, u64* pre, const u64* ct, hipStream_t s);
void launch_gather_sum(const DeviceTables& t, const KsShape& sh, u64* out, const u64* in, size_t in_stride, hipStream_t s);
void launch_moddown_conv(const DeviceTables& t, const KsShape& sh, u64* conv, const u64* accP, const u64* phatinv, const u64* phatmod,
                         hipStream_t s);
void launch_affine_acc(const DeviceTables& t, const KsShape& sh, u64* accQ, const u64* d, const u64* sub, const ScalarSet& cst, int has_cst, int f,
                       const u64* pmod, hipStream_t s);
void launch_moddown_rescale_conv(const DeviceTables& t, const KsShape& sh, u64* conv, const u64* accP, const u64* top, const u64* hatinv,
                                 const u64* hatmod, const u64* mmod, hipStream_t s);
void launch_moddown_rescale_finish(const DeviceTables& t, const KsShape& sh, u64* out, const u64* accQ, const u64* conv, const u64* minv,
                                   hipStream_t s);
void launch_moddown_finish(const DeviceTables& t, const KsShape& sh, u64* out, const u64* accQ, const u64* conv, const u64* pinv,
                           const u64* add0, const u64* add1, const u32* map, const u64* post, hipStream_t s);

}
```

### fhe-linformer_amd/csrc/kernels_elem.hip

```cpp
#include <hip/hip_runtime.h>
#include <cstdlib>
#include <type_traits>
#include "kernels.h"
#include "kernels_elem.h"

namespace fhelin {
namespace {

typedef u64 u64x2 __attribute__((ext_vector_type(2)));

__device__ __forceinline__ Barrett load_barrett(const DeviceTables& t, int limb) {
    Barrett b;
    b.q = t.moduli[limb];
    b.r0 = t.barrett[2 * limb];
    b.r1 = t.barrett[2 * limb + 1];
    return b;
}

template <int OP>
__global__ __launch_bounds__(256) void ew_binary_kernel(DeviceTables t, u64* out, const u64* a, const u64* b, int b_mod,
                                                        int limb_first, int limb_count) {
    const int v = blockIdx.y;
    const int limb = limb_first + v % limb_count;
    const size_t n2 = (size_t)blockIdx.x * 256 + threadIdx.x;
    const size_t row = ((size_t)1 << t.log_n) >> 1;
    const u64x2 x = reinterpret_cast<const u64x2*>(a)[(size_t)v * row + n2];
    const u64x2 y = reinterpret_cast<const u64x2*>(b)[(size_t)(v % b_mod) * row + n2];
    u64x2 r;
    if (OP == 0) {
        const Barrett br = load_barrett(t, limb);
        r.x = mul_mod(x.x, y.x, br);
        r.y = mul_mod(x.y, y.y, br);
    } else if (OP == 1) {
        const u64 q = t.moduli[limb];
        r.x = add_mod(x.x, y.x, q);
        r.y = add_mod(x.y, y.y, q);
    } else {
        const u64 q = t.moduli[limb];
        r.x = sub_mod(x.x, y.x, q);
        r.y = sub_mod(x.y, y.y, q);
    }
    reinterpret_cast<u64x2*>(out)[(size_t)v * row + n2] = r;
}

template <int OP>
__global__ __launch_bounds__(256) void ew_items_kernel(DeviceTables t, EwItems it, int limb_count) {
    const int item = blockIdx.y / it.vecs, v = blockIdx.y % it.vecs;
    const int limb = v % limb_count;
    const size_t n2 = (size_t)blockIdx.x * 256 + threadIdx.x;
    const size_t row = ((size_t)1 << t.log_n) >> 1;
    const u64x2 x = reinterpret_cast<const u64x2*>(it.a[item])[(size_t)v * row + n2];
    u64x2 r = x;
    if (OP != 4 && (OP != 3 || v < it.b_vecs)) {
        const u64x2 y = reinterpret_cast<const u64x2*>(it.b[item])[(size_t)(v % it.b_vecs) * row + n2];
        if (OP == 0) {
            const Barrett br = load_barrett(t, limb);
            r.x = mul_mod(x.x, y.x, br);
            r.y = mul_mod(x.y, y.y, br);
        } else if (OP == 2) {
            const u64 q = t.moduli[limb];
            r.x = sub_mod(x.x, y.x, q);
            r.y = sub_mod(x.y, y.y, q);
        } else {
            const u64 q = t.moduli[limb];
            r.x = add_mod(x.x, y.x, q);
            r.y = add_mod(x.y, y.y, q);
        }
    }
    reinterpret_cast<u64x2*>(it.out[item])[(size_t)v * row + n2] = r;
}

__global__ __launch_bounds__(256) void ew_dot_kernel(DeviceTables t, u64* out, EwItems it, int limb_count) {
    const int v = blockIdx.y;
    const Barrett br = load_barrett(t, v % limb_count);
    const size_t n2 = (size_t)blockIdx.x * 256 + threadIdx.x;
    const size_t row = ((size_t)1 << t.log_n) >> 1;
    Acc128 ax = {0, 0}, ay = {0, 0};
    for (int i = 0; i < it.n; ++i) {
        const u64x2 x = reinterpret_cast<const u64x2*>(it.a[i])[(size_t)v * row + n2];
        const u64x2 y = reinterpret_cast<const u64x2*>(it.b[i])[(size_t)(v % it.b_vecs) * row + n2];
        acc_mac(ax, x.x, y.x);
        acc_mac(ay, x.y, y.y);
    }
    u64x2 r;
    r.x = barrett_reduce128(ax.lo, ax.hi, br);
    r.y = barrett_reduce128(ay.lo, ay.hi, br);
    reinterpret_cast<u64x2*>(out)[(size_t)v * row + n2] = r;
}

template <int NA>
__global__ __launch_bounds__(256) __attribute__((amdgpu_waves_per_eu(NA <= 8 ? 4 : 3))) void ew_dot_groups_kernel(DeviceTables t, EwDotGroups d) {
    const unsigned nx = gridDim.x, nblk = gridDim.x * gridDim.y;
    unsigned id = blockIdx.y * nx + blockIdx.x;
    if ((nblk & 7) == 0) id = (id & 7) * (nblk >> 3) + (id >> 3);
    const int comp = (int)(id & 1);
    const unsigned rest = id >> 1;
    const int xb = (int)(rest % (unsigned)d.nbatch);
    const int bx = (int)((rest / (unsigned)d.nbatch) % nx), tt = (int)((rest / (unsigned)d.nbatch) / nx);
    const Barrett br = load_barrett(t, tt);
    const size_t n2 = (size_t)bx * 256 + threadIdx.x;
    const size_t row = ((size_t)1 << t.log_n) >> 1;
    const size_t op = (size_t)tt * row + n2, oc = (size_t)(comp * d.ell + tt) * row + n2;
    u64x2 a[NA];
#pragma unroll
    for (int b = 0; b < NA; ++b) a[b] = reinterpret_cast<const u64x2*>(d.a[b] + (size_t)xb * d.a_stride[b])[oc];
    if constexpr (NA <= 8) {
        u64x2 w[NA], wn[NA];
#pragma unroll
        for (int b = 0; b < NA; ++b) w[b] = reinterpret_cast<const u64x2*>(d.p[0][b])[op];
        for (int g = 0; g < d.ng; ++g) {
            const int gn = g + 1 < d.ng ? g + 1 : g;
#pragma unroll
            for (int b = 0; b < NA; ++b) wn[b] = reinterpret_cast<const u64x2*>(d.p[gn][b])[op];
            Acc128 x = {0, 0}, y = {0, 0};
            const u32 m = d.pmask[g];
#pragma unroll
            for (int b = 0; b < NA; ++b)
                if (m >> b & 1u) {
                    acc_mac(x, a[b].x, w[b].x);
                    acc_mac(y, a[b].y, w[b].y);
                }
            u64x2 r;
            r.x = barrett_reduce128(x.lo, x.hi, br);
            r.y = barrett_reduce128(y.lo, y.hi, br);
            reinterpret_cast<u64x2*>(d.out[g] + (size_t)xb * d.out_stride[g])[oc] = r;
#pragma unroll
            for (int b = 0; b < NA; ++b) w[b] = wn[b];
        }
    } else {
        for (int g = 0; g < d.ng; ++g) {
            Acc128 x = {0, 0}, y = {0, 0};
            const u32 m = d.pmask[g];
#pragma unroll
            for (int b0 = 0; b0 < NA; b0 += 8) {
                u64x2 w[8];
#pragma unroll
                for (int b = 0; b < 8; ++b) w[b] = reinterpret_cast<const u64x2*>(d.p[g][b0 + b])[op];
#pragma unroll
                for (int b = 0; b < 8; ++b)
                    if (m >> (b0 + b) & 1u) {
                        acc_mac(x, a[b0 + b].x, w[b].x);
                        acc_mac(y, a[b0 + b].y, w[b].y);
                    }
            }
            u64x2 r;
            r.x = barrett_reduce128(x.lo, x.hi, br);
            r.y = barrett_reduce128(y.lo, y.hi, br);
            reinterpret_cast<u64x2*>(d.out[g] + (size_t)xb * d.out_stride[g])[oc] = r;
        }
    }
}

template <int SH>
__device__ __forceinline__ u64 pack_sh(u64 x) { return (x & ((1ull << SH) - 1)) | ((x >> SH) << 32); }
template <int SH>
__device__ __forceinline__ void acc_flush_sh(const Acc30& a, u64& lo, u64& hi) {
    u64 t = lo + a.s0;
    hi += (t < lo);
    lo = t;
    t = lo + (a.s1 << SH);
    hi += (a.s1 >> (64 - SH)) + (t < lo);
    lo = t;
    t = lo + (a.s2 << (2 * SH));
    hi += (a.s2 >> (64 - 2 * SH)) + (t < lo);
    lo = t;
}

#ifndef WSPLIT
#define WSPLIT 1
#endif
template <int I0, int I1, class F>
__device__ __forceinline__ void static_for(F&& f) {
    if constexpr (I0 < I1) {
        f(std::integral_constant<int, I0>{});
        static_for<I0 + 1, I1>(f);
    }
}

template <int SH>
__device__ __forceinline__ void cyclic_body(const DeviceTables& t, const EwCyclic& d, const Barrett& br, u64 (*ml)[256]) {
    constexpr int P = EwCyclic::PERIOD, G = 2;
    const int tt = blockIdx.y;
    const size_t N = (size_t)1 << t.log_n;
    const size_t n = (size_t)blockIdx.x * 256 + threadIdx.x;
    const size_t oc = (size_t)(blockIdx.z * d.ell + tt) * N + n;
    const u32 bm = (u32)(((size_t)tt * N + n) * 8), bc = (u32)(oc * 8);
    auto ld = [](const u64* p, u32 byte_off) -> u64 { return *reinterpret_cast<const u64*>(reinterpret_cast<const char*>(p) + byte_off); };
    {
        u64 mv[P];
#pragma unroll
        for (int j = 0; j < P; ++j) mv[j] = ld(d.m[j], bm);
#pragma unroll
        for (int j = 0; j < P; ++j) ml[j][threadIdx.x] = pack_sh<SH>(mv[j]);
    }
    __builtin_amdgcn_sched_barrier(0);
    u64 a[P];
#pragma unroll
    for (int i = 0; i < P; ++i) a[i] = ld(d.a[i], bc);
#pragma unroll
    for (int i = 0; i < P; ++i) a[i] = i < d.n ? pack_sh<SH>(a[i]) : 0;
#pragma unroll 1
    for (int k = 0; k < P; k += G) {
        u64 lo[G], hi[G];
        Acc30 x[G];
        static_for<0, G>([&](auto I) __attribute__((always_inline)) {
            lo[decltype(I)::value] = hi[decltype(I)::value] = 0;
            x[decltype(I)::value] = Acc30{0, 0, 0};
        });
        static_for<0, P / 8>([&](auto I0) __attribute__((always_inline)) {
            constexpr int i0 = 8 * decltype(I0)::value;
            static_for<i0, i0 + 8>([&](auto I) __attribute__((always_inline)) {
                constexpr int i = decltype(I)::value;
                const u64 w = ml[(i + k) & (P - 1)][threadIdx.x];
                const u32 w0 = (u32)w, w1 = (u32)(w >> 32);
                static_for<0, G>([&](auto Gi) __attribute__((always_inline)) {
                    constexpr int g = decltype(Gi)::value;
                    constexpr int ii = (i - g) & (P - 1);
                    mac30(x[g], (u32)a[ii], (u32)(a[ii] >> 32), w0, w1);
                });
            });
            __builtin_amdgcn_sched_barrier(0);
            if constexpr (SH == 30) {
                static_for<0, G>([&](auto Gi) __attribute__((always_inline)) {
                    constexpr int g = decltype(Gi)::value;
                    acc_flush_sh<30>(x[g], lo[g], hi[g]);
                    x[g] = Acc30{0, 0, 0};
                    if constexpr (i0 == 8) {
                        lo[g] = barrett_reduce128(lo[g], hi[g], br);
                        hi[g] = 0;
                    }
// ... 336 lines not shown
    r.y = barrett_reduce128(x.y, 0, br);
    if (x.x > half) r.x = sub_mod(r.x, qsm, br.q);
    if (x.y > half) r.y = sub_mod(r.y, qsm, br.q);
    reinterpret_cast<u64x2*>(out)[(size_t)v * row + n2] = r;
}

__global__ __launch_bounds__(256) void rescale_finish_kernel(DeviceTables t, u64* out, const u64* c, const u64* lifted, int ell1,
                                                             const u64* qlinv_row) {
    const int v = blockIdx.y;
    const int p = v / ell1, tq = v % ell1;
    const u64 q = t.moduli[tq];
    const u64 w = qlinv_row[2 * tq], ws = qlinv_row[2 * tq + 1];
    const size_t n2 = (size_t)blockIdx.x * 256 + threadIdx.x;
    const size_t row = ((size_t)1 << t.log_n) >> 1;
    const u64x2 x = reinterpret_cast<const u64x2*>(c)[((size_t)p * (ell1 + 1) + tq) * row + n2];
    const u64x2 y = reinterpret_cast<const u64x2*>(lifted)[(size_t)v * row + n2];
    u64x2 r;
    r.x = mul_shoup(sub_mod(x.x, y.x, q), w, ws, q);
    r.y = mul_shoup(sub_mod(x.y, y.y, q), w, ws, q);
    reinterpret_cast<u64x2*>(out)[(size_t)v * row + n2] = r;
}

__global__ __launch_bounds__(256) void reduce_i128_kernel(DeviceTables t, u64* out, const u64* coeffs, int limb_first) {
    const int v = blockIdx.y;
    const Barrett br = load_barrett(t, limb_first + v);
    const size_t n = (size_t)blockIdx.x * 256 + threadIdx.x;
    const size_t N = (size_t)1 << t.log_n;
    u64 lo = coeffs[2 * n], hi = coeffs[2 * n + 1];
    const bool neg = (hi >> 63) != 0;
    if (neg) {
        lo = ~lo + 1;
        hi = ~hi + (lo == 0);
    }
    const u64 h = barrett_reduce128(hi, 0, br);
    u64 r = barrett_reduce128(lo, h, br);
    if (neg) r = neg_mod(r, br.q);
    out[(size_t)v * N + n] = r;
}

inline dim3 grid2(int log_n, int nvec) { return dim3((1u << log_n) / 512, (unsigned)nvec); }

}

void launch_ew_items(const DeviceTables& t, const EwItems& it, int op, int limb_count, hipStream_t s) {
    if (it.n <= 0 || it.vecs <= 0) return;
    const dim3 g = grid2(t.log_n, it.n * it.vecs);
    switch (op) {
        case 0: hipLaunchKernelGGL((ew_items_kernel<0>), g, dim3(256), 0, s, t, it, limb_count); break;
        case 1: hipLaunchKernelGGL((ew_items_kernel<1>), g, dim3(256), 0, s, t, it, limb_count); break;
        case 2: hipLaunchKernelGGL((ew_items_kernel<2>), g, dim3(256), 0, s, t, it, limb_count); break;
        case 4: hipLaunchKernelGGL((ew_items_kernel<4>), g, dim3(256), 0, s, t, it, limb_count); break;
        default: hipLaunchKernelGGL((ew_items_kernel<3>), g, dim3(256), 0, s, t, it, limb_count); break;
    }
}
void launch_ew_dot(const DeviceTables& t, u64* out, const EwItems& it, int limb_count, hipStream_t s) {
    if (it.n <= 0 || it.vecs <= 0) return;
    hipLaunchKernelGGL(ew_dot_kernel, grid2(t.log_n, it.vecs), dim3(256), 0, s, t, out, it, limb_count);
}
void launch_ew_dot_groups(const DeviceTables& t, const EwDotGroups& din, hipStream_t s) {
    if (din.na <= 0 || din.ng <= 0 || din.ell <= 0) return;
    EwDotGroups d = din;
    const int width = d.na <= 8 ? 8 : EwDotGroups::MAX_A;
    const u64* any = d.a[0];
    for (int g = 0; g < d.ng && any == d.a[0]; ++g)
        for (int b = 0; b < d.na; ++b)
            if (d.p[g][b]) {
                any = d.p[g][b];
                break;
            }
    for (int b = d.na; b < width; ++b) {
        d.a[b] = d.a[0];
        d.a_stride[b] = d.a_stride[0];
    }
    for (int g = 0; g < d.ng; ++g) {
        d.pmask[g] = 0;
        for (int b = 0; b < width; ++b) {
            if (b < d.na && d.p[g][b])
                d.pmask[g] |= 1u << b;
            else
                d.p[g][b] = any;
        }
    }
    const int nb = d.nbatch > 0 ? d.nbatch : 1;
    if (d.na <= 8)
        hipLaunchKernelGGL((ew_dot_groups_kernel<8>), grid2(t.log_n, 2 * d.ell * nb), dim3(256), 0, s, t, d);
    else
        hipLaunchKernelGGL((ew_dot_groups_kernel<16>), grid2(t.log_n, 2 * d.ell * nb), dim3(256), 0, s, t, d);
}
void launch_ew_cyclic_dot(const DeviceTables& t, const EwCyclic& din, hipStream_t s) {
    if (din.n <= 0 || din.ell <= 0) return;
    EwCyclic d = din;
    for (int i = d.n; i < EwCyclic::PERIOD; ++i) d.a[i] = d.a[0];
    hipLaunchKernelGGL(ew_cyclic_dot_kernel, dim3((1u << t.log_n) / 256, (unsigned)d.ell, 2), dim3(256), 0, s, t, d);
}
void launch_ew_window_dot(const DeviceTables& t, const EwWindow& d, hipStream_t s) {
    if (d.ell <= 0) return;
    static const int group = [] { const char* e = std::getenv("FHELIN_WINDOW_GROUP"); return e ? std::atoi(e) : 2; }();
    const dim3 g((1u << t.log_n) / 256, (unsigned)d.ell, 2);
    switch (group) {
        case 1: hipLaunchKernelGGL(ew_window_dot_kernel<1>, g, dim3(256), 0, s, t, d); break;
        case 4: hipLaunchKernelGGL(ew_window_dot_kernel<4>, g, dim3(256), 0, s, t, d); break;
        default: hipLaunchKernelGGL(ew_window_dot_kernel<2>, g, dim3(256), 0, s, t, d); break;
    }
}
void launch_ew_mul(const DeviceTables& t, u64* out, const u64* a, const u64* b, int nvec, int b_mod, int limb_first, int limb_count, hipStream_t s) {
    if (nvec <= 0) return;
    hipLaunchKernelGGL((ew_binary_kernel<0>), grid2(t.log_n, nvec), dim3(256), 0, s, t, out, a, b, b_mod, limb_first, limb_count);
}
void launch_ew_add(const DeviceTables& t, u64* out, const u64* a, const u64* b, int nvec, int b_mod, int limb_first, int limb_count, hipStream_t s) {
    if (nvec <= 0) return;
    hipLaunchKernelGGL((ew_binary_kernel<1>), grid2(t.log_n, nvec), dim3(256), 0, s, t, out, a, b, b_mod, limb_first, limb_count);
}
void launch_ew_sub(const DeviceTables& t, u64* out, const u64* a, const u64* b, int nvec, int b_mod, int limb_first, int limb_count, hipStream_t s) {
    if (nvec <= 0) return;
    hipLaunchKernelGGL((ew_binary_kernel<2>), grid2(t.log_n, nvec), dim3(256), 0, s, t, out, a, b, b_mod, limb_first, limb_count);
}
void launch_ew_muladd(const DeviceTables& t, u64* out, const u64* acc, const u64* a, const u64* b, int nvec, int b_mod, int limb_first,
                      int limb_count, hipStream_t s) {
    if (nvec <= 0) return;
    hipLaunchKernelGGL(ew_muladd_kernel, grid2(t.log_n, nvec), dim3(256), 0, s, t, out, acc, a, b, b_mod, limb_first, limb_count);
}
void launch_ew_neg(const DeviceTables& t, u64* out, const u64* a, int nvec, int limb_first, int limb_count, hipStream_t s) {
    if (nvec <= 0) return;
    hipLaunchKernelGGL(ew_neg_kernel, grid2(t.log_n, nvec), dim3(256), 0, s, t, out, a, limb_first, limb_count);
}
void launch_ew_scalar(const DeviceTables& t, u64* out, const u64* a, const ScalarSet& sc, int nvec, int limb_first, int limb_count, hipStream_t s,
                      int in_limbs) {
    if (nvec <= 0) return;
    hipLaunchKernelGGL(ew_scalar_kernel, grid2(t.log_n, nvec), dim3(256), 0, s, t, out, a, sc, limb_first, limb_count, in_limbs);
}
void launch_ew_scaled_diff(const DeviceTables& t, const EwScaledDiff& d, const u64* consts, hipStream_t s) {
    if (d.n <= 0 || d.vecs <= 0 || d.ell <= 0) return;
    hipLaunchKernelGGL(ew_scaled_diff_kernel, grid2(t.log_n, d.n * d.vecs), dim3(256), 0, s, t, d, consts);
}
void launch_ew_addscalar(const DeviceTables& t, u64* out, const u64* a, const ScalarSet& sc, int nvec, int limb_first, int limb_count, hipStream_t s,
                         int add_vecs) {
    if (nvec <= 0) return;
    hipLaunchKernelGGL(ew_addscalar_kernel, grid2(t.log_n, nvec), dim3(256), 0, s, t, out, a, sc, limb_first, limb_count, add_vecs < 0 ? nvec : add_vecs);
}
void launch_ew_lincomb(const DeviceTables& t, u64* out, const LinComb& lc, const u64* scal, int ell, hipStream_t s, int in_limbs) {
    if (lc.n <= 0 || lc.vecs <= 0) return;
    hipLaunchKernelGGL(ew_lincomb_kernel, grid2(t.log_n, lc.vecs), dim3(256), 0, s, t, out, lc, scal, ell, in_limbs);
}
void launch_tensor(const DeviceTables& t, u64* d, const u64* a, const u64* b, int ell, hipStream_t s) {
    hipLaunchKernelGGL(tensor_kernel, grid2(t.log_n, ell), dim3(256), 0, s, t, d, a, b, ell);
}
void launch_tensor_items(const DeviceTables& t, const EwItems& it, int ell, hipStream_t s) {
    if (it.n <= 0) return;
    hipLaunchKernelGGL(tensor_items_kernel, dim3((1u << t.log_n) / 512, (unsigned)ell, (unsigned)it.n), dim3(256), 0, s, t, it, ell);
}
void launch_automorph(const DeviceTables& t, u64* out, const u64* in, const u32* map, int nvec, hipStream_t s) {
    if (nvec <= 0) return;
    hipLaunchKernelGGL(automorph_kernel, grid2(t.log_n, nvec), dim3(256), 0, s, t.log_n, out, in, map);
}
void launch_automorph_pack30(const DeviceTables& t, u64* out, const u64* in, const u32* map, int nvec, hipStream_t s) {
    if (nvec <= 0) return;
    hipLaunchKernelGGL(automorph_pack30_kernel, grid2(t.log_n, nvec), dim3(256), 0, s, t, out, in, map);
}
void launch_rescale_lift(const DeviceTables& t, u64* lifted, const u64* last, int npoly, int ell, const u64* qlmod_row, hipStream_t s) {
    hipLaunchKernelGGL(rescale_lift_kernel, grid2(t.log_n, npoly * (ell - 1)), dim3(256), 0, s, t, lifted, last, ell - 1, qlmod_row);
}
void launch_rescale_finish(const DeviceTables& t, u64* out, const u64* c, const u64* lifted, int npoly, int ell, const u64* qlinv_row,
                           hipStream_t s) {
    hipLaunchKernelGGL(rescale_finish_kernel, grid2(t.log_n, npoly * (ell - 1)), dim3(256), 0, s, t, out, c, lifted, ell - 1, qlinv_row);
}
void launch_modraise(const DeviceTables& t, u64* out, const u64* src, int npoly, int src_limb, int nl, hipStream_t s) {
    hipLaunchKernelGGL(modraise_kernel, grid2(t.log_n, npoly * nl), dim3(256), 0, s, t, out, src, src_limb, nl);
}
void launch_reduce_i128(const DeviceTables& t, u64* out, const u64* coeffs, int limb_first, int nlimbs, hipStream_t s) {
    hipLaunchKernelGGL(reduce_i128_kernel, dim3((1u << t.log_n) / 256, (unsigned)nlimbs), dim3(256), 0, s, t, out, coeffs, limb_first);
// ... 4 lines not shown
```

### fhe-linformer_amd/csrc/kernels_ntt.hip

```cpp
#include <hip/hip_runtime.h>
#include <algorithm>
#include <cstdlib>
#include "kernels.h"

namespace fhelin {

namespace {

struct NttArgs {
    u64* data;
    const u64* src;
    const u64* tw;
    const u64* tw_rows;
    const u64* moduli;
    const u64* ninv;
    const int* limb_tab;
    int tab_len;
    int limb_first;
    int limb_count;
    int log_n;
    int nvec;
    int period;
    int lazy_out;
    int src_group;
    size_t src_group_stride;
    int src_group2;
    size_t src_group2_stride;
    const u64* lift_qlm;
    int lift_limb;
    int vec0;
};

__device__ __forceinline__ size_t src_offset(const NttArgs& a, int vec, int log_n) {
    if (a.src_group > 0) {
        const int g = vec / a.src_group;
        const size_t in = (size_t)(vec % a.src_group) << log_n;
        if (a.src_group2 > 0) return (size_t)(g / a.src_group2) * a.src_group2_stride + (size_t)(g % a.src_group2) * a.src_group_stride + in;
        return (size_t)g * a.src_group_stride + in;
    }
    return (size_t)vec << log_n;
}

constexpr int TILE = 4096;
constexpr int LDS_WORDS = TILE + TILE / 16;

__device__ __forceinline__ int tile_index(int tau, int k, int p) {
    return ((tau >> p) << (p + 4)) | (k << p) | (tau & ((1 << p) - 1));
}
__device__ __forceinline__ int lds_slot(int e) { return e + (e >> 4); }

__device__ __forceinline__ int limb_of(const NttArgs& a, int vec) {
    return a.limb_tab ? a.limb_tab[a.tab_len ? vec % a.tab_len : vec] : a.limb_first + (vec % a.limb_count);
}

typedef u64 u64x2 __attribute__((ext_vector_type(2)));

struct LimbConst {
    u64 q;
    u64 nq;
    u64 q5;
    u32 sh;
    u32 rr;
};

struct RoundTw {
    u64x2 t[15];
};
template <int KB_LO, int KB_HI>
__device__ __forceinline__ void load_round_tw(RoundTw& r, const u64x2* __restrict__ tw, int log_n, int gbase, int hi) {
#pragma unroll
    for (int kb = KB_LO; kb < KB_HI; ++kb) {
        const int m = 1 << (log_n - (gbase + kb) - 1);
        const int tbase = m + (hi << (3 - kb));
#pragma unroll
        for (int j = 0; j < (8 >> kb); ++j) r.t[(8 >> kb) - 1 + j] = tw[tbase + j];
    }
}

__device__ __forceinline__ void load_round_tw_rows(RoundTw& r, const u64x2* __restrict__ trows, int tau) {
#pragma unroll
    for (int s = 0; s < 15; ++s) r.t[s] = trows[s * 256 + tau];
}

template <int KB, bool LAZY>
__device__ __forceinline__ void fwd_stage(u64 (&x)[16], const RoundTw& tw, const LimbConst& c) {
#pragma unroll
    for (int k0 = 0; k0 < 16; ++k0) {
        if (k0 & (1 << KB)) continue;
        const int k1 = k0 | (1 << KB);
        const u64x2 w = tw.t[(8 >> KB) - 1 + (k0 >> (KB + 1))];
        const u64 X = LAZY ? x[k0] : csub_mask(x[k0], c.q5);
#if defined(FHELIN_BFLY15)
        const u64 T = mul_shoup_lazy5(x[k1], w.x, w.y, c.nq);
        x[k0] = X + T;
        x[k1] = X + c.q5 - T;
#else
        const u64 A = mul_shoup_lazy5_add(x[k1], w.x, w.y, c.nq, X);
        x[k0] = A;
        x[k1] = shl1_add(X, c.q5) - A;
#endif
    }
}
template <int KB_LO, int KB_HI, bool LAZY>
__device__ __forceinline__ void fwd_round(u64 (&x)[16], const RoundTw& tw, const LimbConst& c) {
    if constexpr (KB_LO < KB_HI) {
        fwd_stage<KB_HI - 1, LAZY>(x, tw, c);
        fwd_round<KB_LO, KB_HI - 1, LAZY>(x, tw, c);
    }
}

constexpr int lazy_coef(int s, int c0) { return s == 0 ? c0 : 5 << (s - 1); }

template <int KB, bool FINAL, bool LAZY, int S, int C0>
__device__ __forceinline__ void inv_stage(u64 (&x)[16], const RoundTw& tw, const LimbConst& c, const u64* __restrict__ ninv) {
    const u64 B = c.q * (u64)lazy_coef(S, C0);
    if constexpr (FINAL) {
        const u64 ni = ninv[0], nis = ninv[1], wn = ninv[2], wns = ninv[3];
#pragma unroll
        for (int k0 = 0; k0 < 16; ++k0) {
            if (k0 & (1 << KB)) continue;
            const int k1 = k0 | (1 << KB);
            const u64 X = x[k0], Y = x[k1];
            if (LAZY) {
                x[k0] = csub_mask(reduce_lazy_2q(mul_shoup_lazy5(X + Y, ni, nis, c.nq), c.q, c.sh, c.rr), c.q);
                x[k1] = csub_mask(reduce_lazy_2q(mul_shoup_lazy5(X + B - Y, wn, wns, c.nq), c.q, c.sh, c.rr), c.q);
            } else {
                x[k0] = csub_mask(reduce_lazy_2q(mul_shoup_lazy5(X + Y, ni, nis, c.nq), c.q, c.sh, c.rr), c.q);
                x[k1] = csub_mask(reduce_lazy_2q(mul_shoup_lazy5(X + c.q5 - Y, wn, wns, c.nq), c.q, c.sh, c.rr), c.q);
            }
        }
    } else {
#pragma unroll
        for (int k0 = 0; k0 < 16; ++k0) {
            if (k0 & (1 << KB)) continue;
            const int k1 = k0 | (1 << KB);
            const u64x2 w = tw.t[(8 >> KB) - 1 + (k0 >> (KB + 1))];
            const u64 X = x[k0], Y = x[k1];
            if (LAZY) {
                x[k0] = X + Y;
                x[k1] = mul_shoup_lazy5(X + B - Y, w.x, w.y, c.nq);
            } else {
                x[k0] = csub_mask(X + Y, c.q5);
                x[k1] = mul_shoup_lazy5(X + c.q5 - Y, w.x, w.y, c.nq);
            }
        }
    }
}
template <int KB_LO, int KB_HI, bool LAST, bool LAZY, int S0 = 0, int C0 = 1>
__device__ __forceinline__ void inv_round(u64 (&x)[16], const RoundTw& tw, const LimbConst& c, const u64* __restrict__ ninv) {
    if constexpr (KB_LO < KB_HI) {
        inv_stage<KB_LO, (LAST && KB_LO == KB_HI - 1), LAZY, S0, C0>(x, tw, c, ninv);
        inv_round<KB_LO + 1, KB_HI, LAST, LAZY, S0 + 1, C0>(x, tw, c, ninv);
    }
}

__device__ __forceinline__ void exchange(u64 (&x)[16], u64* lds, int tau, int p_from, int p_to, bool sync_first) {
    if (sync_first) __syncthreads();
#pragma unroll
    for (int k = 0; k < 16; ++k) lds[lds_slot(tile_index(tau, k, p_from))] = x[k];
    __syncthreads();
#pragma unroll
    for (int k = 0; k < 16; ++k) x[k] = lds[lds_slot(tile_index(tau, k, p_to))];
}

__device__ __forceinline__ LimbConst limb_const(const NttArgs& a, int limb) {
    LimbConst c;
    c.q = a.moduli[limb];
    c.nq = 0 - c.q;
    c.q5 = 5 * c.q;
    c.sh = (u32)a.ninv[8 * limb + 4];
    c.rr = (u32)a.ninv[8 * limb + 5];
    return c;
}
#if defined(FHELIN_NTT_FORCE_PATH)
template <bool INVERSE> __device__ __forceinline__ bool lazy_prime(u64) { return FHELIN_NTT_FORCE_PATH; }
#else
template <bool INVERSE> __device__ __forceinline__ bool lazy_prime(u64 q) { return q < (1ull << (INVERSE ? 53 : 57)); }
#endif

template <int A, bool INVERSE, bool LAZY, bool LIFT>
__device__ __forceinline__ void cols_body(const NttArgs& a, u64* lds, int vec, int tile, int limb, const LimbConst& c) {
    constexpr int LOGCW = 12 - A;
    constexpr int CW = 1 << LOGCW;
    constexpr int LOGN = A + 8;
    constexpr int NFULL = A / 4;
    constexpr int REM = A % 4;
    const u64x2* tw = reinterpret_cast<const u64x2*>(a.tw) + ((size_t)limb << LOGN);
    u64* base = a.data + ((size_t)vec << LOGN) + tile * CW;
    const u64* sbase = (LIFT ? a.src + ((size_t)(vec / a.limb_count) << LOGN) : a.src + src_offset(a, vec, LOGN)) + tile * CW;
    const int tau = threadIdx.x;
    u64 x[16];

    auto goff = [](int e) { return ((e >> LOGCW) << 8) | (e & (CW - 1)); };

    if (!INVERSE) {
        constexpr int P0 = LOGCW + A - 4;
#pragma unroll
        for (int k = 0; k < 16; ++k) x[k] = sbase[goff(tile_index(tau, k, P0))];
        if constexpr (LIFT) {
            const u64 half = a.moduli[a.lift_limb] >> 1, qlm = a.lift_qlm[limb];
#pragma unroll
            for (int k = 0; k < 16; ++k) {
                const u64 r = csub_mask(x[k], c.q);
                x[k] = x[k] > half ? sub_mod(r, qlm, c.q) : r;
            }
        }
        RoundTw rt, rn;
        load_round_tw<0, 4>(rt, tw, LOGN, 8 + P0 - LOGCW, tau >> P0);
        fwd_round<0, 4, LAZY>(x, rt, c);
        int p_prev = P0;
        if constexpr (NFULL >= 2) {
            constexpr int P1 = LOGCW + A - 8;
            load_round_tw<0, 4>(rn, tw, LOGN, 8 + P1 - LOGCW, tau >> P1);
            exchange(x, lds, tau, p_prev, P1, false);
            fwd_round<0, 4, LAZY>(x, rn, c);
            p_prev = P1;
        }
        if constexpr (REM > 0) {
            constexpr int PR = LOGCW;
            load_round_tw<0, REM>(rt, tw, LOGN, 8, tau >> PR);
            exchange(x, lds, tau, p_prev, PR, NFULL >= 2);
            fwd_round<0, REM, LAZY>(x, rt, c);
            p_prev = PR;
        }
        constexpr int PL = REM > 0 ? LOGCW : (NFULL >= 2 ? LOGCW + A - 8 : P0);
        (void)p_prev;
#pragma unroll
        for (int k = 0; k < 16; ++k) base[goff(tile_index(tau, k, PL))] = x[k];
    } else {
        const u64* ninv = a.ninv + 8 * limb;
        constexpr int P0 = LOGCW;
#pragma unroll
        for (int k = 0; k < 16; ++k) x[k] = sbase[goff(tile_index(tau, k, P0))];
        RoundTw rt, rn;
        load_round_tw<0, 4>(rt, tw, LOGN, 8, tau >> P0);
        inv_round<0, 4, (NFULL == 1 && REM == 0), LAZY, 0, 2>(x, rt, c, ninv);
        int p_prev = P0;
        if constexpr (NFULL >= 2) {
            constexpr int P1 = LOGCW + 4;
            load_round_tw<0, 4>(rn, tw, LOGN, 8 + 4, tau >> P1);
            exchange(x, lds, tau, p_prev, P1, false);
            inv_round<0, 4, (REM == 0), LAZY, 4, 2>(x, rn, c, ninv);
            p_prev = P1;
        }
        if constexpr (REM > 0) {
            constexpr int PR = 8;
            load_round_tw<4 - REM, 4>(rt, tw, LOGN, 8 + PR - LOGCW, tau >> PR);
            exchange(x, lds, tau, p_prev, PR, NFULL >= 2);
            inv_round<4 - REM, 4, true, LAZY, 4 * NFULL, 2>(x, rt, c, ninv);
            p_prev = PR;
        }
        constexpr int PL = REM > 0 ? 8 : (NFULL >= 2 ? LOGCW + 4 : P0);
        (void)p_prev;
#pragma unroll
        for (int k = 0; k < 16; ++k) base[goff(tile_index(tau, k, PL))] = x[k];
    }
}

template <int A, bool INVERSE, bool LIFT = false>
__global__ __launch_bounds__(256) __attribute__((amdgpu_waves_per_eu(LIFT ? 3 : 4))) void ntt_cols_kernel(NttArgs a) {
    constexpr int LOGTILES = A - 4;
    __shared__ u64 lds[LDS_WORDS];
    const int vec = a.vec0 + (blockIdx.x >> LOGTILES);
    const int tile = blockIdx.x & ((1 << LOGTILES) - 1);
    const int limb = limb_of(a, vec);
    if (limb < 0) return;
    const LimbConst c = limb_const(a, limb);
    if (lazy_prime<INVERSE>(c.q))
        cols_body<A, INVERSE, true, LIFT>(a, lds, vec, tile, limb, c);
    else
        cols_body<A, INVERSE, false, LIFT>(a, lds, vec, tile, limb, c);
}

template <bool INVERSE, bool LAZY, bool EPI>
__device__ __forceinline__ void rows_body(const NttArgs& a, u64* lds, int vec, int tile, int limb, const LimbConst& c,
                                          const NttEpilogue* ep) {
    const int log_n = a.log_n;
    const u64x2* tw = reinterpret_cast<const u64x2*>(a.tw) + ((size_t)limb << log_n);
    const u64x2* trows = reinterpret_cast<const u64x2*>(a.tw_rows) + (((size_t)limb << (log_n - 12)) + tile) * (15 * 256);
    u64* base = a.data + ((size_t)vec << log_n) + ((size_t)tile << 12);
    const u64* sbase = a.src + src_offset(a, vec, log_n) + ((size_t)tile << 12);
    const int tau = threadIdx.x;
    u64 x[16];

    if (!INVERSE) {
#pragma unroll
        for (int k = 0; k < 16; ++k) x[k] = sbase[tile_index(tau, k, 4)];
        RoundTw rt, rn;
        load_round_tw<0, 4>(rt, tw, log_n, 4, (tile << 4) | (tau >> 4));
        fwd_round<0, 4, LAZY>(x, rt, c);
        load_round_tw_rows(rn, trows, tau);
        exchange(x, lds, tau, 4, 0, false);
        fwd_round<0, 4, LAZY>(x, rn, c);
        [[maybe_unused]] u64 av[16];
        [[maybe_unused]] int ell = 0, t = 0, poly = 0;
        if constexpr (EPI) {
            ell = ep->ell;
            t = vec % ell;
            poly = vec / ell;
            const u64* acc = ep->acc + (size_t)poly * ep->acc_poly_stride + ((size_t)t << log_n) + ((size_t)tile << 12);
#pragma unroll
            for (int k = 0; k < 16; ++k) av[k] = acc[tile_index(tau, k, 8)];
        }
        if constexpr (EPI) {
#pragma unroll
            for (int k = 0; k < 16; ++k) x[k] = reduce_lazy_2q(x[k], c.q, c.sh, c.rr);
        } else if (!(LAZY && a.lazy_out && c.q < (1ull << 53))) {
#pragma unroll
            for (int k = 0; k < 16; ++k)
                x[k] = csub_mask(reduce_lazy_2q(x[k], c.q, c.sh, c.rr), c.q);
        }
#if defined(FHELIN_ROWS_DIRECT_STORE)
        if constexpr (!EPI) {
#pragma unroll
            for (int k = 0; k < 16; k += 2) {
                u64x2 v;
                v.x = x[k];
                v.y = x[k + 1];
                reinterpret_cast<u64x2*>(base + 16 * tau)[k >> 1] = v;
            }
            return;
        }
#endif
        exchange(x, lds, tau, 0, 8, true);
        if constexpr (EPI) {
            const int bi = poly >> 1, comp = poly & 1;
            const size_t n = (size_t)1 << log_n;
            const u64 w = ep->w[2 * t], ws = ep->w[2 * t + 1];
            const u64 q2 = 2 * c.q;
#pragma unroll
            for (int k = 0; k < 16; ++k) x[k] = mul_shoup(av[k] + q2 - x[k], w, ws, c.q);
            const u64* add = comp == 0 ? ep->add0 : ep->add1;
            if (add) {
                add += (size_t)bi * ep->add_stride + (size_t)t * n + ((size_t)tile << 12);
#pragma unroll
                for (int k = 0; k < 16; ++k) x[k] = add_mod(x[k], add[tile_index(tau, k, 8)], c.q);
            }
            const size_t row_off = (size_t)(comp * ell + t) * n;
            const u64* post = ep->post ? ep->post + (size_t)bi * ep->post_stride + row_off : nullptr;
            u64* out = ep->out + (size_t)bi * ep->out_stride + row_off;
            const u32* im = ep->per_row ? ep->invmap_row[bi] : ep->invmap;
            if (im) {
#pragma unroll
                for (int k = 0; k < 16; ++k) {
                    const size_t j = im[((size_t)tile << 12) + tile_index(tau, k, 8)];
                    u64 r = x[k];
                    if (post) r = add_mod(r, post[j], c.q);
                    out[j] = r;
                }
            } else {
                out += (size_t)tile << 12;
                if (post) {
                    post += (size_t)tile << 12;
#pragma unroll
                    for (int k = 0; k < 16; ++k) x[k] = add_mod(x[k], post[tile_index(tau, k, 8)], c.q);
                }
#pragma unroll
                for (int k = 0; k < 16; ++k) out[tile_index(tau, k, 8)] = x[k];
            }
        } else {
#pragma unroll
            for (int k = 0; k < 16; ++k) base[tile_index(tau, k, 8)] = x[k];
        }
    } else {
#pragma unroll
        for (int k = 0; k < 16; ++k) x[k] = sbase[tile_index(tau, k, 8)];
        RoundTw rt, rn;
        load_round_tw_rows(rt, trows, tau);
        exchange(x, lds, tau, 8, 0, false);
        inv_round<0, 4, false, LAZY, 0, 1>(x, rt, c, nullptr);
        load_round_tw<0, 4>(rn, tw, log_n, 4, (tile << 4) | (tau >> 4));
        exchange(x, lds, tau, 0, 4, true);
        inv_round<0, 4, false, LAZY, 4, 1>(x, rn, c, nullptr);
        if (LAZY) {
#pragma unroll
            for (int k = 0; k < 16; ++k) x[k] = reduce_lazy_2q(x[k], c.q, c.sh, c.rr);
        }
#pragma unroll
        for (int k = 0; k < 16; ++k) base[tile_index(tau, k, 4)] = x[k];
    }
}

template <bool INVERSE, bool EPI = false>
__global__ __launch_bounds__(256) __attribute__((amdgpu_waves_per_eu(4))) void ntt_rows_kernel(NttArgs a, NttEpilogue ep) {
    __shared__ u64 lds[LDS_WORDS];
    const int logtiles = a.log_n - 12;
    int lid = blockIdx.x;
    const int nblk = gridDim.x;
    if ((nblk & 7) == 0) lid = (lid & 7) * (nblk >> 3) + (lid >> 3);
    int vec, tile;
    if (a.period > 0) {
        const int nper = a.nvec / a.period;
        const int rep = lid % nper, r = lid / nper;
        tile = r & ((1 << logtiles) - 1);
        vec = a.vec0 + rep * a.period + (r >> logtiles);
    } else {
        vec = a.vec0 + (lid >> logtiles);
        tile = lid & ((1 << logtiles) - 1);
    }
    const int limb = limb_of(a, vec);
    if (limb < 0) return;
    const LimbConst c = limb_const(a, limb);
    if (lazy_prime<INVERSE>(c.q))
        rows_body<INVERSE, true, EPI>(a, lds, vec, tile, limb, c, &ep);
    else
        rows_body<INVERSE, false, EPI>(a, lds, vec, tile, limb, c, &ep);
}

template <int A>
void launch_cols(const NttArgs& a, bool inverse, int blocks, hipStream_t s) {
    if (inverse)
        hipLaunchKernelGGL((ntt_cols_kernel<A, true>), dim3(blocks), dim3(256), 0, s, a);
    else if (a.lift_qlm)
        hipLaunchKernelGGL((ntt_cols_kernel<A, false, true>), dim3(blocks), dim3(256), 0, s, a);
    else
        hipLaunchKernelGGL((ntt_cols_kernel<A, false>), dim3(blocks), dim3(256), 0, s, a);
}

}

static void launch_ntt_impl(const DeviceTables& t, const LimbBatch& b, bool inverse, const NttEpilogue* ep, hipStream_t s);

void launch_ntt(const DeviceTables& t, const LimbBatch& b, bool inverse, hipStream_t s) { launch_ntt_impl(t, b, inverse, nullptr, s); }
void launch_ntt_epilogue(const DeviceTables& t, const LimbBatch& b, const NttEpilogue& ep, hipStream_t s) {
    launch_ntt_impl(t, b, false, &ep, s);
}

static void launch_ntt_impl(const DeviceTables& t, const LimbBatch& b, bool inverse, const NttEpilogue* ep, hipStream_t s) {
    if (b.nvec <= 0) return;
    NttArgs a;
    a.data = b.data;
    a.src = b.src ? b.src : b.data;
    a.src_group = b.src ? b.src_group : 0;
    a.src_group_stride = b.src_group_stride;
    a.src_group2 = (b.src && b.src_group > 0) ? b.src_group2 : 0;
    a.src_group2_stride = b.src_group2_stride;
    a.lazy_out = (!inverse && b.lazy_out) ? 1 : 0;
    a.lift_qlm = (!inverse && b.src && b.lift_limb >= 0) ? b.lift_qlm : nullptr;
    a.lift_limb = b.lift_limb;
    a.tw = inverse ? t.tw_inv : t.tw_fwd;
    a.tw_rows = inverse ? t.tw_rows_inv : t.tw_rows_fwd;
    a.moduli = t.moduli;
    a.ninv = t.ninv;
    a.limb_tab = b.limb_tab;
    a.tab_len = b.tab_len;
    a.limb_first = b.limb_first;
    a.limb_count = b.limb_count > 0 ? b.limb_count : 1;
    a.log_n = t.log_n;
    a.nvec = b.nvec;
    const int per = b.limb_tab ? b.tab_len : a.limb_count;
    a.period = (per > 0 && per < b.nvec && b.nvec % per == 0) ? per : 0;
    const int A = t.log_n - 8;
    a.vec0 = 0;
    static const int chunk_mb = [] {
        const char* e = std::getenv("FHELIN_NTT_CHUNK_MB");
        return e ? std::atoi(e) : 0;
    }();
    int chunk = b.nvec;
    if (chunk_mb > 0 && !ep) {
        const size_t vec_bytes = (size_t)8 << t.log_n;
        const int want = (int)std::max<size_t>(1, ((size_t)chunk_mb << 20) / vec_bytes);
        if (b.nvec > want + want / 2) {
            const int per = a.period > 0 ? a.period : 1;
            chunk = std::max(per, want / per * per);
        }
    }
    const int nvec_all = b.nvec, period_all = a.period;
    const u64* src_all = a.src;
    const int sg = a.src_group, sg2 = a.src_group2;
    for (int v0 = 0; v0 < nvec_all; v0 += chunk) {
        a.vec0 = v0;
        a.nvec = std::min(chunk, nvec_all - v0);
        a.period = (period_all > 0 && a.nvec % period_all == 0 && a.nvec > period_all) ? period_all : 0;
        a.src = src_all;
        a.src_group = sg;
        a.src_group2 = sg2;
        const int blocks = a.nvec << (t.log_n - 12);
        auto cols = [&]() {
            switch (A) {
                case 4: launch_cols<4>(a, inverse, blocks, s); break;
                case 5: launch_cols<5>(a, inverse, blocks, s); break;
                case 6: launch_cols<6>(a, inverse, blocks, s); break;
                case 7: launch_cols<7>(a, inverse, blocks, s); break;
                case 8: launch_cols<8>(a, inverse, blocks, s); break;
                case 9: launch_cols<9>(a, inverse, blocks, s); break;
                default: break;
            }
        };
        if (!inverse) {
            cols();
            a.src = a.data;
            a.src_group = 0;
            a.src_group2 = 0;
            if (ep)
                hipLaunchKernelGGL((ntt_rows_kernel<false, true>), dim3(blocks), dim3(256), 0, s, a, *ep);
            else
                hipLaunchKernelGGL((ntt_rows_kernel<false, false>), dim3(blocks), dim3(256), 0, s, a, NttEpilogue());
        } else {
            hipLaunchKernelGGL((ntt_rows_kernel<true, false>), dim3(blocks), dim3(256), 0, s, a, NttEpilogue());
            a.src = a.data;
            a.src_group = 0;
            a.src_group2 = 0;
            cols();
        }
    }
}

}
```

Before: 240.4.

## Fold INTT N^-1 scaling into base-conversion tables and add Montgomery dot-groups path

For key-switching inverse NTTs, the final multiply by N^-1 is skipped, and N^-1 is folded into the hat-inverse tables used by modup, moddown and moddown-rescale base conversion. This removes one modular multiply per coefficient from each key-switch INTT. Separately, the plaintext dot-groups kernel gains a REDC variant: it converts the activation operands with a Shoup multiply, accumulates them in 30-bit packed form, and finishes with Montgomery reduction instead of Barrett. Both paths are on by default behind env flags, and they add new kernel template instantiations plus extra precomputed tables.

Result: faster. 237.6 (median of 6 runs) (-1.2%).

```diff
diff --git a/fhe-linformer_amd/csrc/context.cpp b/fhe-linformer_amd/csrc/context.cpp
--- a/fhe-linformer_amd/csrc/context.cpp
+++ b/fhe-linformer_amd/csrc/context.cpp
@@ -221,6 +221,16 @@
 template const double* Context::upload_table<double>(const std::vector<double>&);
 
 static u64 mont_r(u64 m) { return (u64)((((u128)1) << 64) % m); }
+
+static std::vector<u64> times_ninv(const std::vector<u64>& pairs, const std::vector<u64>& mods, u64 N) {
+    std::vector<u64> r(pairs.size());
+    for (size_t i = 0; i < mods.size(); ++i) {
+        const u64 m = mods[i];
+        r[2 * i] = h_mulmod(pairs[2 * i], h_invmod(N % m, m), m);
+        r[2 * i + 1] = h_shoup(r[2 * i], m);
+    }
+    return r;
+}
 
 static u64 prod_mod(const std::vector<u64>& ms, int skip, u64 t) {
     u64 r = 1 % t;
@@ -312,6 +322,8 @@
         if (const char* e = std::getenv("FHELIN_ASYNC")) async_lanes = std::atoi(e) != 0;
         if (const char* e = std::getenv("FHELIN_FUSE_MODDOWN")) fuse_moddown = std::atoi(e) != 0;
         if (const char* e = std::getenv("FHELIN_FUSE_FINISH")) fuse_finish = std::atoi(e) != 0;
+        if (const char* e = std::getenv("FHELIN_INTT_FOLD_NINV")) fold_ninv = std::atoi(e) != 0;
+        if (const char* e = std::getenv("FHELIN_DOT_GROUPS_REDC")) dot_groups_redc = std::atoi(e) != 0;
         if (const char* e = std::getenv("FHELIN_HOST_ENCODE")) host_encode = std::atoi(e) != 0;
         if (const char* e = std::getenv("FHELIN_FUSE_GATHER")) fuse_gather = std::atoi(e) != 0;
         if (const char* e = std::getenv("FHELIN_FUSE_LIFT")) fuse_lift = std::atoi(e) != 0;
@@ -411,6 +423,7 @@
             pinv[2 * t + 1] = h_shoup(inv, qt);
         }
         d_phatinv = upload_table(phatinv);
+        d_phatinv_ninv = upload_table(K > 0 ? times_ninv(phatinv, chain.p, (u64)N) : phatinv);
         d_phatmod = upload_table(phatmod);
         d_pinv = upload_table(pinv);
         std::vector<u64> pmod(2 * (L + 1));
@@ -461,6 +474,7 @@
             }
         }
         lt.up_hatinv = upload_table(hatinv);
+        lt.up_hatinv_ninv = upload_table(times_ninv(hatinv, std::vector<u64>(chain.q.begin(), chain.q.begin() + ell), (u64)N));
         lt.up_hatmod = upload_table(hatmod);
         lt.up_hatmod_r2 = upload_table(hatmod2);
         lt.ext_limb_tab = upload_table(tab);
@@ -487,6 +501,9 @@
                 minv[2 * t + 1] = h_shoup(inv, qt);
             }
             lt.md_hatinv = upload_table(mhi);
+            std::vector<u64> mb(chain.p.begin(), chain.p.end());
+            mb.push_back(ql);
+            lt.md_hatinv_ninv = upload_table(times_ninv(mhi, mb, (u64)N));
             lt.md_hatmod = upload_table(mhm);
             lt.md_minv = upload_table(minv);
             lt.md_mmod = upload_table(mmod);
diff --git a/fhe-linformer_amd/csrc/context.h b/fhe-linformer_amd/csrc/context.h
--- a/fhe-linformer_amd/csrc/context.h
+++ b/fhe-linformer_amd/csrc/context.h
@@ -92,10 +92,12 @@
     int ell = 0;
     int beta = 0;
     const u64* up_hatinv = nullptr;
+    const u64* up_hatinv_ninv = nullptr;
     const u64* up_hatmod = nullptr;
     const u64* up_hatmod_r2 = nullptr;
     const int* ext_limb_tab = nullptr;
     const u64* md_hatinv = nullptr;
+    const u64* md_hatinv_ninv = nullptr;
     const u64* md_hatmod = nullptr;
     const u64* md_minv = nullptr;
     const u64* md_mmod = nullptr;
@@ -172,6 +174,7 @@
     void upload_async(u64* dst, const u64* src, size_t words);
 
     const u64* d_phatinv = nullptr;
+    const u64* d_phatinv_ninv = nullptr;
     const u64* d_phatmod = nullptr;
     const u64* d_pinv = nullptr;
     const u64* d_pmod = nullptr;
@@ -201,6 +204,15 @@
     bool fuse_gather = true;
     bool fuse_lift = true;
     bool lds_digits = true;
+    bool fold_ninv = true;
+    bool dot_groups_redc = true;
+    void ks_intt(LimbBatch b) {
+        b.no_ninv = fold_ninv;
+        ntt(b, true);
+    }
+    const u64* up_hatinv_ks(const LevelTables& lt) const { return fold_ninv ? lt.up_hatinv_ninv : lt.up_hatinv; }
+    const u64* md_hatinv_ks(const LevelTables& lt) const { return fold_ninv ? lt.md_hatinv_ninv : lt.md_hatinv; }
+    const u64* phatinv_ks() const { return fold_ninv ? d_phatinv_ninv : d_phatinv; }
     struct FftDev {
         const u32* rot = nullptr;
         const double* ksi = nullptr;
diff --git a/fhe-linformer_amd/csrc/evaluator.cpp b/fhe-linformer_amd/csrc/evaluator.cpp
--- a/fhe-linformer_amd/csrc/evaluator.cpp
+++ b/fhe-linformer_amd/csrc/evaluator.cpp
@@ -167,10 +167,10 @@
             ib.src_group = ell;
             ib.src_group_stride = c_stride;
         }
-        c_.ntt(ib, true);
+        c_.ks_intt(ib);
     }
     u64* ext = c_.dalloc<u64>((size_t)Bu * lt.beta * nt * N);
-    launch_modup_conv(c_.dt, shu, ext, cc, c_ntt, lt.up_hatinv, lt.up_hatmod_r2, s);
+    launch_modup_conv(c_.dt, shu, ext, cc, c_ntt, c_.up_hatinv_ks(lt), lt.up_hatmod_r2, s);
     LimbBatch eb{ext, Bu * lt.beta * nt, lt.ext_limb_tab, 0, 1};
     eb.tab_len = lt.beta * nt;
     eb.lazy_out = true;
@@ -178,9 +178,9 @@
     u64* accQ = c_.dalloc<u64>((size_t)B * 2 * ell * N);
     u64* accP = c_.dalloc<u64>((size_t)B * 2 * K * N);
     launch_ks_inner(c_.dt, sh, accQ, accP, ext, key ? key->d : nullptr, c_ntt, s);
-    c_.ntt(LimbBatch{accP, B * 2 * K, nullptr, L1, K}, true);
+    c_.ks_intt(LimbBatch{accP, B * 2 * K, nullptr, L1, K});
     u64* conv = c_.dalloc<u64>((size_t)B * 2 * ell * N);
-    launch_moddown_conv(c_.dt, sh, conv, accP, c_.d_phatinv, c_.d_phatmod, s);
+    launch_moddown_conv(c_.dt, sh, conv, accP, c_.phatinv_ks(), c_.d_phatmod, s);
     const bool identity = !map && !rows;
     if (c_.fuse_moddown || (c_.fuse_finish && identity)) {
         NttEpilogue ep;
@@ -306,10 +306,10 @@
                 ib.src_group = ell;
                 ib.src_group_stride = ctw;
             }
-            c_.ntt(ib, true);
+            c_.ks_intt(ib);
         }
         u64* ext = c_.dalloc<u64>((size_t)B * lt.beta * nt * N);
-        launch_modup_conv(c_.dt, sh, ext, cc, base + pn, lt.up_hatinv, lt.up_hatmod, s);
+        launch_modup_conv(c_.dt, sh, ext, cc, base + pn, c_.up_hatinv_ks(lt), lt.up_hatmod, s);
         LimbBatch eb{ext, B * lt.beta * nt, lt.ext_limb_tab, 0, 1};
         eb.tab_len = lt.beta * nt;
         eb.lazy_out = true;
@@ -325,9 +325,9 @@
             c0sum = c_.dalloc<u64>((size_t)B * ell * N);
             launch_gather_sum(c_.dt, sh, c0sum, base, ctw, s);
         }
-        c_.ntt(LimbBatch{accP, B * 2 * K, nullptr, L1, K}, true);
+        c_.ks_intt(LimbBatch{accP, B * 2 * K, nullptr, L1, K});
         u64* conv = c_.dalloc<u64>((size_t)B * 2 * ell * N);
-        launch_moddown_conv(c_.dt, sh, conv, accP, c_.d_phatinv, c_.d_phatmod, s);
+        launch_moddown_conv(c_.dt, sh, conv, accP, c_.phatinv_ks(), c_.d_phatmod, s);
         c_.ntt(LimbBatch{conv, B * 2 * ell, nullptr, 0, ell}, false);
         launch_moddown_finish(c_.dt, sh, o[0]->d, accQ, conv, c_.d_pinv, c0sum, nullptr, nullptr, base, s);
         launch_ok("rotate_sum_batch");
@@ -469,10 +469,10 @@
                 ib.src_group = ell;
                 ib.src_group_stride = ctw;
             }
-            c_.ntt(ib, true);
+            c_.ks_intt(ib);
         }
         u64* ext = c_.dalloc<u64>((size_t)B * lt.beta * nt * N);
-        launch_modup_conv(c_.dt, sh, ext, cc, base + pn, lt.up_hatinv, lt.up_hatmod, s);
+        launch_modup_conv(c_.dt, sh, ext, cc, base + pn, c_.up_hatinv_ks(lt), lt.up_hatmod, s);
         LimbBatch eb{ext, B * lt.beta * nt, lt.ext_limb_tab, 0, 1};
         eb.tab_len = lt.beta * nt;
         eb.lazy_out = true;
@@ -486,25 +486,25 @@
         if (!merged) {
             pre = c_.dalloc<u64>((size_t)B * ctw);
             launch_hoist_addends(c_.dt, sh, h, pre, base, s);
-            c_.ntt(LimbBatch{accP, B * 2 * K, nullptr, L1, K}, true);
+            c_.ks_intt(LimbBatch{accP, B * 2 * K, nullptr, L1, K});
             conv = c_.dalloc<u64>((size_t)B * 2 * ell * N);
-            launch_moddown_conv(c_.dt, sh, conv, accP, c_.d_phatinv, c_.d_phatmod, s);
+            launch_moddown_conv(c_.dt, sh, conv, accP, c_.phatinv_ks(), c_.d_phatmod, s);
             c_.ntt(LimbBatch{conv, B * 2 * ell, nullptr, 0, ell}, false);
             launch_moddown_finish(c_.dt, sh, o[0]->d, accQ, conv, c_.d_pinv, nullptr, nullptr, nullptr, pre, s);
         } else {
             h.acc = accQ;
             h.pmod = c_.d_pmod;
             launch_hoist_addends(c_.dt, sh, h, nullptr, base, s);
-            c_.ntt(LimbBatch{accP, B * 2 * K, nullptr, L1, K}, true);
+            c_.ks_intt(LimbBatch{accP, B * 2 * K, nullptr, L1, K});
             top = c_.dalloc<u64>((size_t)B * 2 * N);
             {
                 LimbBatch tb{top, B * 2, nullptr, ell - 1, 1, accQ + (size_t)(ell - 1) * N};
                 tb.src_group = 1;
                 tb.src_group_stride = pn;
-                c_.ntt(tb, true);
+                c_.ks_intt(tb);
             }
             conv = c_.dalloc<u64>((size_t)B * 2 * (ell - 1) * N);
-            launch_moddown_rescale_conv(c_.dt, sh, conv, accP, top, lt.md_hatinv, lt.md_hatmod, lt.md_mmod, s);
+            launch_moddown_rescale_conv(c_.dt, sh, conv, accP, top, c_.md_hatinv_ks(lt), lt.md_hatmod, lt.md_mmod, s);
             moddown_rescale_finish(sh, o[0]->d, accQ, conv, lt.md_minv);
         }
         launch_ok("hoisted_dot_rows");
@@ -566,10 +566,10 @@
             LimbBatch ib{cc, R * ell, nullptr, 0, ell, base + pn};
             ib.src_group = ell;
             ib.src_group_stride = ctw;
-            c_.ntt(ib, true);
+            c_.ks_intt(ib);
         }
         u64* ext = c_.dalloc<u64>((size_t)R * lt.beta * nt * N);
-        launch_modup_conv(c_.dt, up, ext, cc, base + pn, lt.up_hatinv, lt.up_hatmod, s);
+        launch_modup_conv(c_.dt, up, ext, cc, base + pn, c_.up_hatinv_ks(lt), lt.up_hatmod, s);
         LimbBatch eb{ext, R * lt.beta * nt, lt.ext_limb_tab, 0, 1};
         eb.tab_len = lt.beta * nt;
         eb.lazy_out = true;
@@ -596,9 +596,9 @@
             c0sum = c_.dalloc<u64>((size_t)ell * N);
             launch_gather_sum(c_.dt, sh, c0sum, base, 0, s);
         }
-        c_.ntt(LimbBatch{accP, 2 * K, nullptr, L1, K}, true);
+        c_.ks_intt(LimbBatch{accP, 2 * K, nullptr, L1, K});
         u64* conv = c_.dalloc<u64>((size_t)2 * ell * N);
-        launch_moddown_conv(c_.dt, sh, conv, accP, c_.d_phatinv, c_.d_phatmod, s);
+        launch_moddown_conv(c_.dt, sh, conv, accP, c_.phatinv_ks(), c_.d_phatmod, s);
         c_.ntt(LimbBatch{conv, 2 * ell, nullptr, 0, ell}, false);
         CtPtr o = new_ct(2, ell, chunk[0]->deg, chunk[0]->scale, chunk[0]->slots);
         launch_moddown_finish(c_.dt, sh, o->d, accQ, conv, c_.d_pinv, c0sum, nullptr, nullptr, nullptr, s);
@@ -680,10 +680,10 @@
                 ib.src_group2 = R;
                 ib.src_group2_stride = row_stride;
             }
-            c_.ntt(ib, true);
+            c_.ks_intt(ib);
         }
         u64* ext = c_.dalloc<u64>((size_t)B * R * lt.beta * nt * N);
-        launch_modup_conv(c_.dt, up, ext, cc, base + pn, lt.up_hatinv, lt.up_hatmod, s);
+        launch_modup_conv(c_.dt, up, ext, cc, base + pn, c_.up_hatinv_ks(lt), lt.up_hatmod, s);
         LimbBatch eb{ext, B * R * lt.beta * nt, lt.ext_limb_tab, 0, 1};
         eb.tab_len = lt.beta * nt;
         eb.lazy_out = true;
@@ -705,9 +705,9 @@
         u64* accQ = c_.dalloc<u64>((size_t)B * 2 * ell * N);
         u64* accP = c_.dalloc<u64>((size_t)B * 2 * K * N);
         launch_ks_inner_multi(c_.dt, sh, accQ, accP, ext, base + pn, s);
-        c_.ntt(LimbBatch{accP, B * 2 * K, nullptr, L1, K}, true);
+        c_.ks_intt(LimbBatch{accP, B * 2 * K, nullptr, L1, K});
         u64* conv = c_.dalloc<u64>((size_t)B * 2 * ell * N);
-        launch_moddown_conv(c_.dt, sh, conv, accP, c_.d_phatinv, c_.d_phatmod, s);
+        launch_moddown_conv(c_.dt, sh, conv, accP, c_.phatinv_ks(), c_.d_phatmod, s);
         c_.ntt(LimbBatch{conv, B * 2 * ell, nullptr, 0, ell}, false);
         std::vector<CtPtr> o = new_ct_batch(B, 2, ell, f->deg, f->scale, f->slots);
         launch_moddown_finish(c_.dt, sh, o[0]->d, accQ, conv, c_.d_pinv, nullptr, nullptr, nullptr, nullptr, s);
@@ -998,10 +998,10 @@
                 ib.src_group = ell;
                 ib.src_group_stride = ctw;
             }
-            c_.ntt(ib, true);
+            c_.ks_intt(ib);
         }
         u64* ext = c_.dalloc<u64>((size_t)B * lt.beta * nt * N);
-        launch_modup_conv(c_.dt, up, ext, cc, base + pn, lt.up_hatinv, lt.up_hatmod_r2, s);
+        launch_modup_conv(c_.dt, up, ext, cc, base + pn, c_.up_hatinv_ks(lt), lt.up_hatmod_r2, s);
         LimbBatch eb{ext, B * lt.beta * nt, lt.ext_limb_tab, 0, 1};
         eb.tab_len = lt.beta * nt;
         eb.lazy_out = true;
@@ -1038,9 +1038,9 @@
                                     base + pn + (size_t)i * ctw, s);
                 }
         KsShape dn{ell, K, c_.alpha, lt.beta, L1, rows, 0, ctw, 0, 0};
-        c_.ntt(LimbBatch{accP, rows * 2 * K, nullptr, L1, K}, true);
+        c_.ks_intt(LimbBatch{accP, rows * 2 * K, nullptr, L1, K});
         u64* conv = c_.dalloc<u64>((size_t)rows * 2 * ell * N);
-        launch_moddown_conv(c_.dt, dn, conv, accP, c_.d_phatinv, c_.d_phatmod, s);
+        launch_moddown_conv(c_.dt, dn, conv, accP, c_.phatinv_ks(), c_.d_phatmod, s);
         c_.ntt(LimbBatch{conv, rows * 2 * ell, nullptr, 0, ell}, false);
         std::vector<CtPtr> o = new_ct_batch(rows, 2, ell, xs[lo]->deg, xs[lo]->scale, xs[lo]->slots);
         if (one_chunk) {
@@ -1267,6 +1267,7 @@
         dest[g]->scale = f->scale * sf;
         dest[g]->slots = f->slots;
     }
+    d.redc = c_.dot_groups_redc;
     launch_ew_dot_groups(c_.dt, d, c_.stream);
     launch_ok("dot_plain_groups");
     c_.stats.ct_pt_mult += terms;
@@ -1330,6 +1331,7 @@
             dest[x][g]->slots = f->slots;
         }
     }
+    d.redc = c_.dot_groups_redc;
     launch_ew_dot_groups(c_.dt, d, c_.stream);
     launch_ok("dot_plain_groups_batch");
     c_.stats.ct_pt_mult += terms * nb;
@@ -1610,10 +1612,10 @@
                 ib.src_group = ell;
                 ib.src_group_stride = 3 * pn;
             }
-            c_.ntt(ib, true);
+            c_.ks_intt(ib);
         }
         u64* ext = c_.dalloc<u64>((size_t)B * lt.beta * nt * N);
-        launch_modup_conv(c_.dt, sh, ext, cc, c_ntt, lt.up_hatinv, lt.up_hatmod_r2, s);
+        launch_modup_conv(c_.dt, sh, ext, cc, c_ntt, c_.up_hatinv_ks(lt), lt.up_hatmod_r2, s);
         LimbBatch eb{ext, B * lt.beta * nt, lt.ext_limb_tab, 0, 1};
         eb.tab_len = lt.beta * nt;
         eb.lazy_out = true;
@@ -1623,16 +1625,16 @@
         launch_ks_inner(c_.dt, sh, accQ, accP, ext, relin_key->d, c_ntt, s);
         launch_affine_acc(c_.dt, sh, accQ, d[0]->d, sadj.empty() ? nullptr : sadj[0]->d, cst, cadd != 0.0 ? 1 : 0, f, c_.d_pmod, s);
         if (f == 2) launch_ew_add(c_.dt, accP, accP, accP, B * 2 * K, B * 2 * K, L1, K, s);
-        c_.ntt(LimbBatch{accP, B * 2 * K, nullptr, L1, K}, true);
+        c_.ks_intt(LimbBatch{accP, B * 2 * K, nullptr, L1, K});
         u64* top = c_.dalloc<u64>((size_t)B * 2 * N);
         {
             LimbBatch tb{top, B * 2, nullptr, ell - 1, 1, accQ + (size_t)(ell - 1) * N};
             tb.src_group = 1;
             tb.src_group_stride = pn;
-            c_.ntt(tb, true);
+            c_.ks_intt(tb);
         }
         u64* conv = c_.dalloc<u64>((size_t)B * 2 * (ell - 1) * N);
-        launch_moddown_rescale_conv(c_.dt, sh, conv, accP, top, lt.md_hatinv, lt.md_hatmod, lt.md_mmod, s);
+        launch_moddown_rescale_conv(c_.dt, sh, conv, accP, top, c_.md_hatinv_ks(lt), lt.md_hatmod, lt.md_mmod, s);
         std::vector<CtPtr> o = new_ct_batch(B, 2, ell - 1, 1, 0, x[first]->slots);
         moddown_rescale_finish(sh, o[0]->d, accQ, conv, lt.md_minv);
         launch_ok("mult_affine_rescale_batch");
diff --git a/fhe-linformer_amd/csrc/kernels.h b/fhe-linformer_amd/csrc/kernels.h
--- a/fhe-linformer_amd/csrc/kernels.h
+++ b/fhe-linformer_amd/csrc/kernels.h
@@ -21,6 +21,7 @@
     bool lazy_out = false;
     const u64* lift_qlm = nullptr;
     int lift_limb = -1;
+    bool no_ninv = false;
 };
 
 struct DeviceTables {
diff --git a/fhe-linformer_amd/csrc/kernels_elem.h b/fhe-linformer_amd/csrc/kernels_elem.h
--- a/fhe-linformer_amd/csrc/kernels_elem.h
+++ b/fhe-linformer_amd/csrc/kernels_elem.h
@@ -66,6 +66,7 @@
     size_t a_stride[MAX_A] = {};
     size_t out_stride[MAX_G] = {};
     u32 pmask[MAX_G] = {};
+    bool redc = true;
 };
 void launch_ew_dot_groups(const DeviceTables& t, const EwDotGroups& d, hipStream_t s);
 struct EwCyclic {
diff --git a/fhe-linformer_amd/csrc/kernels_elem.hip b/fhe-linformer_amd/csrc/kernels_elem.hip
--- a/fhe-linformer_amd/csrc/kernels_elem.hip
+++ b/fhe-linformer_amd/csrc/kernels_elem.hip
@@ -88,7 +88,35 @@
     reinterpret_cast<u64x2*>(out)[(size_t)v * row + n2] = r;
 }
 
-template <int NA>
+template <bool REDC>
+__device__ __forceinline__ u64 dot_operand(u64 x, u64 q, u64 r, u64 rs) {
+    if constexpr (REDC) return pack30(mul_shoup(x, r, rs, q));
+    else return x;
+}
+template <bool REDC>
+struct DotAcc {
+    Acc128 w = {0, 0};
+    Acc30 s = {0, 0, 0};
+};
+template <bool REDC>
+__device__ __forceinline__ void dot_mac(DotAcc<REDC>& acc, u64 a, u64 p) {
+    if constexpr (REDC) mac30(acc.s, (u32)a, (u32)(a >> 32), (u32)p & 0x3FFFFFFFu, (u32)(p >> 30));
+    else acc_mac(acc.w, a, p);
+}
+template <bool REDC>
+__device__ __forceinline__ void dot_flush(DotAcc<REDC>& acc) {
+    if constexpr (REDC) {
+        acc30_flush(acc.s, acc.w.lo, acc.w.hi);
+        acc.s = Acc30{0, 0, 0};
+    }
+}
+template <bool REDC>
+__device__ __forceinline__ u64 dot_finish(const DotAcc<REDC>& acc, const Barrett& br, u64 qinv) {
+    if constexpr (REDC) return redc128(acc.w.lo, acc.w.hi, br.q, qinv);
+    else return barrett_reduce128(acc.w.lo, acc.w.hi, br);
+}
+
+template <int NA, bool REDC>
 __global__ __launch_bounds__(256) __attribute__((amdgpu_waves_per_eu(NA <= 8 ? 4 : 3))) void ew_dot_groups_kernel(DeviceTables t, EwDotGroups d) {
     const unsigned nx = gridDim.x, nblk = gridDim.x * gridDim.y;
     unsigned id = blockIdx.y * nx + blockIdx.x;
@@ -98,12 +126,21 @@
     const int xb = (int)(rest % (unsigned)d.nbatch);
     const int bx = (int)((rest / (unsigned)d.nbatch) % nx), tt = (int)((rest / (unsigned)d.nbatch) / nx);
     const Barrett br = load_barrett(t, tt);
+    const u64 qinv = REDC ? t.qinv[tt] : 0;
     const size_t n2 = (size_t)bx * 256 + threadIdx.x;
     const size_t row = ((size_t)1 << t.log_n) >> 1;
     const size_t op = (size_t)tt * row + n2, oc = (size_t)(comp * d.ell + tt) * row + n2;
     u64x2 a[NA];
 #pragma unroll
     for (int b = 0; b < NA; ++b) a[b] = reinterpret_cast<const u64x2*>(d.a[b] + (size_t)xb * d.a_stride[b])[oc];
+    if constexpr (REDC) {
+        const u64 r = t.mont[2 * tt], rs = t.mont[2 * tt + 1];
+#pragma unroll
+        for (int b = 0; b < NA; ++b) {
+            a[b].x = dot_operand<REDC>(a[b].x, br.q, r, rs);
+            a[b].y = dot_operand<REDC>(a[b].y, br.q, r, rs);
+        }
+    }
     if constexpr (NA <= 8) {
         u64x2 w[NA], wn[NA];
 #pragma unroll
@@ -112,24 +149,26 @@
             const int gn = g + 1 < d.ng ? g + 1 : g;
 #pragma unroll
             for (int b = 0; b < NA; ++b) wn[b] = reinterpret_cast<const u64x2*>(d.p[gn][b])[op];
-            Acc128 x = {0, 0}, y = {0, 0};
+            DotAcc<REDC> x, y;
             const u32 m = d.pmask[g];
 #pragma unroll
             for (int b = 0; b < NA; ++b)
                 if (m >> b & 1u) {
-                    acc_mac(x, a[b].x, w[b].x);
-                    acc_mac(y, a[b].y, w[b].y);
+                    dot_mac(x, a[b].x, w[b].x);
+                    dot_mac(y, a[b].y, w[b].y);
                 }
+            dot_flush(x);
+            dot_flush(y);
             u64x2 r;
-            r.x = barrett_reduce128(x.lo, x.hi, br);
-            r.y = barrett_reduce128(y.lo, y.hi, br);
+            r.x = dot_finish(x, br, qinv);
+            r.y = dot_finish(y, br, qinv);
             reinterpret_cast<u64x2*>(d.out[g] + (size_t)xb * d.out_stride[g])[oc] = r;
 #pragma unroll
             for (int b = 0; b < NA; ++b) w[b] = wn[b];
         }
     } else {
         for (int g = 0; g < d.ng; ++g) {
-            Acc128 x = {0, 0}, y = {0, 0};
+            DotAcc<REDC> x, y;
             const u32 m = d.pmask[g];
 #pragma unroll
             for (int b0 = 0; b0 < NA; b0 += 8) {
@@ -139,13 +178,15 @@
 #pragma unroll
                 for (int b = 0; b < 8; ++b)
                     if (m >> (b0 + b) & 1u) {
-                        acc_mac(x, a[b0 + b].x, w[b].x);
-                        acc_mac(y, a[b0 + b].y, w[b].y);
+                        dot_mac(x, a[b0 + b].x, w[b].x);
+                        dot_mac(y, a[b0 + b].y, w[b].y);
                     }
+                dot_flush(x);
+                dot_flush(y);
             }
             u64x2 r;
-            r.x = barrett_reduce128(x.lo, x.hi, br);
-            r.y = barrett_reduce128(y.lo, y.hi, br);
+            r.x = dot_finish(x, br, qinv);
+            r.y = dot_finish(y, br, qinv);
             reinterpret_cast<u64x2*>(d.out[g] + (size_t)xb * d.out_stride[g])[oc] = r;
         }
     }
@@ -648,10 +689,19 @@
         }
     }
     const int nb = d.nbatch > 0 ? d.nbatch : 1;
-    if (d.na <= 8)
-        hipLaunchKernelGGL((ew_dot_groups_kernel<8>), grid2(t.log_n, 2 * d.ell * nb), dim3(256), 0, s, t, d);
-    else
-        hipLaunchKernelGGL((ew_dot_groups_kernel<16>), grid2(t.log_n, 2 * d.ell * nb), dim3(256), 0, s, t, d);
+    const bool redc = d.redc;
+    const dim3 g = grid2(t.log_n, 2 * d.ell * nb);
+    if (d.na <= 8) {
+        if (redc)
+            hipLaunchKernelGGL((ew_dot_groups_kernel<8, true>), g, dim3(256), 0, s, t, d);
+        else
+            hipLaunchKernelGGL((ew_dot_groups_kernel<8, false>), g, dim3(256), 0, s, t, d);
+    } else {
+        if (redc)
+            hipLaunchKernelGGL((ew_dot_groups_kernel<16, true>), g, dim3(256), 0, s, t, d);
+        else
+            hipLaunchKernelGGL((ew_dot_groups_kernel<16, false>), g, dim3(256), 0, s, t, d);
+    }
 }
 void launch_ew_cyclic_dot(const DeviceTables& t, const EwCyclic& din, hipStream_t s) {
     if (din.n <= 0 || din.ell <= 0) return;
diff --git a/fhe-linformer_amd/csrc/kernels_ntt.hip b/fhe-linformer_amd/csrc/kernels_ntt.hip
--- a/fhe-linformer_amd/csrc/kernels_ntt.hip
+++ b/fhe-linformer_amd/csrc/kernels_ntt.hip
@@ -29,6 +29,7 @@
     const u64* lift_qlm;
     int lift_limb;
     int vec0;
+    int no_ninv;
 };
 
 __device__ __forceinline__ size_t src_offset(const NttArgs& a, int vec, int log_n) {
@@ -178,7 +179,7 @@
 template <bool INVERSE> __device__ __forceinline__ bool lazy_prime(u64 q) { return q < (1ull << (INVERSE ? 53 : 57)); }
 #endif
 
-template <int A, bool INVERSE, bool LAZY, bool LIFT>
+template <int A, bool INVERSE, bool LAZY, bool LIFT, bool NONINV>
 __device__ __forceinline__ void cols_body(const NttArgs& a, u64* lds, int vec, int tile, int limb, const LimbConst& c) {
     constexpr int LOGCW = 12 - A;
     constexpr int CW = 1 << LOGCW;
@@ -228,26 +229,27 @@
 #pragma unroll
         for (int k = 0; k < 16; ++k) base[goff(tile_index(tau, k, PL))] = x[k];
     } else {
+        constexpr bool FIN = !NONINV;
         const u64* ninv = a.ninv + 8 * limb;
         constexpr int P0 = LOGCW;
 #pragma unroll
         for (int k = 0; k < 16; ++k) x[k] = sbase[goff(tile_index(tau, k, P0))];
         RoundTw rt, rn;
         load_round_tw<0, 4>(rt, tw, LOGN, 8, tau >> P0);
-        inv_round<0, 4, (NFULL == 1 && REM == 0), LAZY, 0, 2>(x, rt, c, ninv);
+        inv_round<0, 4, FIN && (NFULL == 1 && REM == 0), LAZY, 0, 2>(x, rt, c, ninv);
         int p_prev = P0;
         if constexpr (NFULL >= 2) {
             constexpr int P1 = LOGCW + 4;
             load_round_tw<0, 4>(rn, tw, LOGN, 8 + 4, tau >> P1);
             exchange(x, lds, tau, p_prev, P1, false);
-            inv_round<0, 4, (REM == 0), LAZY, 4, 2>(x, rn, c, ninv);
+            inv_round<0, 4, FIN && (REM == 0), LAZY, 4, 2>(x, rn, c, ninv);
             p_prev = P1;
         }
         if constexpr (REM > 0) {
             constexpr int PR = 8;
             load_round_tw<4 - REM, 4>(rt, tw, LOGN, 8 + PR - LOGCW, tau >> PR);
             exchange(x, lds, tau, p_prev, PR, NFULL >= 2);
-            inv_round<4 - REM, 4, true, LAZY, 4 * NFULL, 2>(x, rt, c, ninv);
+            inv_round<4 - REM, 4, FIN, LAZY, 4 * NFULL, 2>(x, rt, c, ninv);
             p_prev = PR;
         }
         constexpr int PL = REM > 0 ? 8 : (NFULL >= 2 ? LOGCW + 4 : P0);
@@ -257,7 +259,7 @@
     }
 }
 
-template <int A, bool INVERSE, bool LIFT = false>
+template <int A, bool INVERSE, bool LIFT = false, bool NONINV = false>
 __global__ __launch_bounds__(256) __attribute__((amdgpu_waves_per_eu(LIFT ? 3 : 4))) void ntt_cols_kernel(NttArgs a) {
     constexpr int LOGTILES = A - 4;
     __shared__ u64 lds[LDS_WORDS];
@@ -267,9 +269,9 @@
     if (limb < 0) return;
     const LimbConst c = limb_const(a, limb);
     if (lazy_prime<INVERSE>(c.q))
-        cols_body<A, INVERSE, true, LIFT>(a, lds, vec, tile, limb, c);
+        cols_body<A, INVERSE, true, LIFT, NONINV>(a, lds, vec, tile, limb, c);
     else
-        cols_body<A, INVERSE, false, LIFT>(a, lds, vec, tile, limb, c);
+        cols_body<A, INVERSE, false, LIFT, NONINV>(a, lds, vec, tile, limb, c);
 }
 
 template <bool INVERSE, bool LAZY, bool EPI>
@@ -409,7 +411,9 @@
 
 template <int A>
 void launch_cols(const NttArgs& a, bool inverse, int blocks, hipStream_t s) {
-    if (inverse)
+    if (inverse && a.no_ninv)
+        hipLaunchKernelGGL((ntt_cols_kernel<A, true, false, true>), dim3(blocks), dim3(256), 0, s, a);
+    else if (inverse)
         hipLaunchKernelGGL((ntt_cols_kernel<A, true>), dim3(blocks), dim3(256), 0, s, a);
     else if (a.lift_qlm)
         hipLaunchKernelGGL((ntt_cols_kernel<A, false, true>), dim3(blocks), dim3(256), 0, s, a);
@@ -436,6 +440,7 @@
     a.src_group2 = (b.src && b.src_group > 0) ? b.src_group2 : 0;
     a.src_group2_stride = b.src_group2_stride;
     a.lazy_out = (!inverse && b.lazy_out) ? 1 : 0;
+    a.no_ninv = (inverse && b.no_ninv) ? 1 : 0;
     a.lift_qlm = (!inverse && b.src && b.lift_limb >= 0) ? b.lift_qlm : nullptr;
     a.lift_limb = b.lift_limb;
     a.tw = inverse ? t.tw_inv : t.tw_fwd;
```
